# rlorenzo/facet

Hardware: AMD Instinct MI355X
Metric: images/sec whole-node (TOPIQ+SAMP+CLIP+InsightFace ensemble), 1024² batch (higher is better)
Workload: dtype f32

## Files before the change

### facet_amd/_lib.py

```python
import ctypes as C
import importlib.util
import os
import sys
import threading

import numpy as np

_HERE = os.path.dirname(os.path.abspath(__file__))
LIB_PATH = os.environ.get("FACET_AMD_LIB") or os.path.join(_HERE, "libfacet_engine.so")

FE_MODEL_TOPIQ, FE_MODEL_CLIP, FE_MODEL_SAMP, FE_MODEL_U2NETP, FE_MODEL_AESTHETIC, FE_MODEL_VLM = range(6)
FE_MODEL_SCRFD, FE_MODEL_ARCFACE = 5, 6
FE_RECORD_FLOATS = 789
FE_GRAPH_FACE_DET, FE_GRAPH_FACE_LMK, FE_GRAPH_FACE_REC = 0, 1, 2
FE_FACE_FLOATS = 739
FE_STATS_DOUBLES = 264
FILTERS = {"lanczos": 1, "bilinear": 2, "bicubic": 3}
FE_PRECISION_RES32 = 16
FE_PRECISION_SPLIT3 = 32
PRECISION = {"f32": 0, "fp32": 0, "float32": 0, "bf16": 1, "bfloat16": 1, "f16": 2, "fp16": 2, "float16": 2, "half": 2,
             "bf16+r32": 1 | FE_PRECISION_RES32, "f16+r32": 2 | FE_PRECISION_RES32, "f16x3": 2 | FE_PRECISION_RES32 | FE_PRECISION_SPLIT3}
PRECISION_NAME = {0: "f32", 1: "bf16", 2: "f16", 1 | FE_PRECISION_RES32: "bf16+r32", 2 | FE_PRECISION_RES32: "f16+r32",
                  2 | FE_PRECISION_RES32 | FE_PRECISION_SPLIT3: "f16x3"}
ACT = {"none": 0, None: 0, "relu": 1, "gelu": 2, "sigmoid": 3, "softplus": 5}


class EngineError(RuntimeError):
    pass


class EngineCapacityError(EngineError):
    """The batch did not fit (device memory, arena, KV cache): FE_ERR_CAPACITY, raised by the padded-batch image path only
    (vlm_preprocess_rgb, vlm_encode_preprocessed, vlm_prefill with pad). Fewer images at a time may fit. jpeg_encode / face_thumbnails raise it when the
    caller's `cap` is too small for an image."""


FE_ERR_CAPACITY = -4


_lib = None
_lib_lock = threading.Lock()

_f32p = C.POINTER(C.c_float)
_u8p = C.POINTER(C.c_uint8)
_i64p = C.POINTER(C.c_int64)

SIGNATURES = {
    "fe_create": (C.c_int, [C.c_int, C.c_size_t, C.POINTER(C.c_void_p)]),
    "fe_destroy": (None, [C.c_void_p]),
    "fe_last_error": (C.c_char_p, [C.c_void_p]),
    "fe_version": (C.c_char_p, []),
    "fe_sync": (C.c_int, [C.c_void_p]),
    "fe_set_microbatch": (C.c_int, [C.c_void_p, C.c_int]),
    "fe_set_precision": (C.c_int, [C.c_void_p, C.c_int]),
    "fe_model_precision": (C.c_int, [C.c_void_p, C.c_int]),
    "fe_dev_alloc": (C.c_int, [C.c_void_p, C.c_size_t, C.POINTER(C.c_void_p)]),
    "fe_dev_free": (C.c_int, [C.c_void_p, C.c_void_p]),
    "fe_memcpy_h2d": (C.c_int, [C.c_void_p, C.c_void_p, C.c_void_p, C.c_size_t]),
    "fe_memcpy_d2h": (C.c_int, [C.c_void_p, C.c_void_p, C.c_void_p, C.c_size_t]),
    "fe_timer_start": (C.c_int, [C.c_void_p]),
    "fe_timer_stop": (C.c_int, [C.c_void_p, _f32p]),
    "fe_profile_enable": (C.c_int, [C.c_void_p, C.c_int]),
    "fe_profile_count": (C.c_int, [C.c_void_p]),
    "fe_profile_get": (C.c_int, [C.c_void_p, C.c_int, C.c_char_p, C.c_int, C.POINTER(C.c_double),
                                 C.POINTER(C.c_double), _f32p]),
    "fe_flops_reset": (C.c_int, [C.c_void_p]),
    "fe_flops_get": (C.c_int, [C.c_void_p, C.POINTER(C.c_double)]),
    "fe_flops_get_executed": (C.c_int, [C.c_void_p, C.POINTER(C.c_double)]),
    "fe_flops_get_half": (C.c_int, [C.c_void_p, C.POINTER(C.c_double)]),
    "fe_weights_begin": (C.c_int, [C.c_void_p, C.c_int]),
    "fe_weights_set": (C.c_int, [C.c_void_p, C.c_int, C.c_char_p, _f32p, _i64p, C.c_int]),
    "fe_weights_commit": (C.c_int, [C.c_void_p, C.c_int]),
    "fe_model_unload": (C.c_int, [C.c_void_p, C.c_int]),
    "fe_model_loaded": (C.c_int, [C.c_void_p, C.c_int]),
    "fe_op_conv2d": (C.c_int, [C.c_void_p, _f32p, C.c_int, C.c_int, C.c_int, C.c_int, _f32p, C.c_int, C.c_int,
                               C.c_int, _f32p, _f32p, _f32p, C.c_int, C.c_int, C.c_int, C.c_int, C.c_int, _f32p]),
    "fe_op_topiq_gate64": (C.c_int, [C.c_void_p, _f32p, C.c_int, C.c_int, C.c_int, _f32p, _f32p, _f32p, _f32p, _f32p, C.c_float,
                                     _f32p, _f32p, C.c_int, C.c_int, _f32p]),
    "fe_op_conv3x3_c64": (C.c_int, [C.c_void_p, _f32p, C.c_int, C.c_int, C.c_int, _f32p, _f32p, _f32p, C.c_int, _f32p, _f32p, _f32p,
                                    _f32p, _f32p]),
    "fe_op_maxpool2d": (C.c_int, [C.c_void_p, _f32p, C.c_int, C.c_int, C.c_int, C.c_int, C.c_int, C.c_int,
                                  C.c_int, C.c_int, _f32p]),
    "fe_op_bilinear": (C.c_int, [C.c_void_p, _f32p, C.c_int, C.c_int, C.c_int, C.c_int, C.c_int, C.c_int, _f32p]),
    "fe_op_adaptive_avgpool": (C.c_int, [C.c_void_p, _f32p, C.c_int, C.c_int, C.c_int, C.c_int, C.c_int, C.c_int,
                                         _f32p]),
    "fe_op_layernorm": (C.c_int, [C.c_void_p, _f32p, C.c_int, C.c_int, _f32p, _f32p, C.c_float, _f32p]),
    "fe_op_vlm_select": (C.c_int, [C.c_void_p, _f32p, C.c_int, C.c_int, C.POINTER(C.c_int32), _f32p]),
    "fe_set_conv_variant": (C.c_int, [C.c_void_p, C.c_int]),
    "fe_bench_conv": (C.c_int, [C.c_void_p] + [C.c_int] * 12 + [_f32p]),
    "fe_topiq_configure": (C.c_int, [C.c_void_p, C.c_int, C.c_int]),
    "fe_topiq_f32_below": (C.c_int, [C.c_void_p, C.c_longlong]),
    "fe_topiq_feature_shape": (C.c_int, [C.c_int, C.c_int, C.c_int, C.POINTER(C.c_int)]),
    "fe_ensemble_select": (C.c_int, [C.c_void_p, C.c_int]),
    "fe_ensemble_score_dev": (C.c_int, [C.c_void_p, C.c_void_p, C.c_int, C.c_int, C.c_int, C.c_int, C.c_void_p, C.c_int,
                                        C.POINTER(C.c_int)]),
    "fe_topiq_features": (C.c_int, [C.c_void_p, C.c_void_p, C.c_int, C.c_int, C.c_int, C.c_int, C.c_int, _f32p]),
    "fe_topiq_score": (C.c_int, [C.c_void_p, C.c_void_p, C.c_int, C.c_int, C.c_int, C.c_int, _f32p]),
    "fe_clip_encode_image": (C.c_int, [C.c_void_p, C.c_void_p, C.c_int, C.c_int, _f32p, _f32p, _f32p]),
    "fe_resize_u8": (C.c_int, [C.c_void_p, C.c_void_p, C.c_int, C.c_int, C.c_int, C.c_int, C.c_int, C.c_int, C.c_int,
                               C.c_void_p]),
    "fe_clip_encode_images": (C.c_int, [C.c_void_p, C.c_void_p, C.c_int, C.c_int, C.c_int, C.c_int, _f32p, _f32p, _f32p]),
    "fe_samp_score_images": (C.c_int, [C.c_void_p, C.c_void_p, C.c_int, C.c_int, C.c_int, C.c_int, C.c_int, _f32p,
                                       _f32p, _f32p]),
    "fe_clip_encode_text": (C.c_int, [C.c_void_p, C.POINTER(C.c_int32), C.c_int, C.c_int, _f32p]),
    "fe_tag_similarities": (C.c_int, [C.c_void_p, _f32p, C.c_int, _f32p, C.c_int, C.c_int, _f32p]),
    "fe_vlm_configure": (C.c_int, [C.c_void_p, C.c_int, C.c_int, C.c_int, C.c_float, C.c_float, C.POINTER(C.c_int)]),
    "fe_vlm_dims": (C.c_int, [C.c_void_p, C.POINTER(C.c_int)]),
    "fe_vlm_prefill": (C.c_int, [C.c_void_p, C.POINTER(C.c_int32), C.POINTER(C.c_int32), C.c_int, C.c_int, C.c_int, C.POINTER(C.c_int32), _f32p]),
    "fe_vlm_decode_step": (C.c_int, [C.c_void_p, C.POINTER(C.c_int32), C.POINTER(C.c_int32), C.c_int, C.POINTER(C.c_int32), _f32p]),
    "fe_vlm_vision_configure": (C.c_int, [C.c_void_p, C.c_int, C.POINTER(C.c_int), C.c_int]),
    "fe_vlm_encode_images": (C.c_int, [C.c_void_p, _f32p, C.c_int, C.POINTER(C.c_int32), C.POINTER(C.c_int32), C.POINTER(C.c_int32), C.c_int,
                                       C.POINTER(C.c_int32), C.c_int, _f32p]),
    "fe_vlm_prefill_images": (C.c_int, [C.c_void_p, C.POINTER(C.c_int32), C.POINTER(C.c_int32), C.c_int, C.c_int, C.c_int, C.POINTER(C.c_int32), C.c_int,
                                        C.POINTER(C.c_int32), _f32p]),
    "fe_vlm_generate": (C.c_int, [C.c_void_p, C.POINTER(C.c_int32), C.POINTER(C.c_int32), C.c_int, C.c_int, C.POINTER(C.c_int32)]),
    "fe_vlm_generate_scored": (C.c_int, [C.c_void_p, C.POINTER(C.c_int32), C.POINTER(C.c_int32), C.c_int, C.c_int, C.POINTER(C.c_int32), _f32p]),
    "fe_vlm_last_logprobs": (C.c_int, [C.c_void_p, _f32p]),
    "fe_vlm_preprocess_rgb": (C.c_int, [C.c_void_p, C.c_void_p, C.c_int, C.POINTER(C.c_int32), _f32p, _f32p, _f32p]),
    "fe_vlm_encode_preprocessed": (C.c_int, [C.c_void_p, C.POINTER(C.c_int32), C.POINTER(C.c_int32), C.POINTER(C.c_int32), C.c_int,
                                             C.POINTER(C.c_int32), C.c_int, _f32p]),
    "fe_vlm_vision_dims": (C.c_int, [C.c_void_p, C.POINTER(C.c_int)]),
    "fe_vlm3_configure": (C.c_int, [C.c_void_p, C.c_int, C.c_int, C.c_int, C.c_float, C.c_float, C.POINTER(C.c_int), C.c_int, C.POINTER(C.c_int), C.c_int]),
    "fe_vlm3_encode_images": (C.c_int, [C.c_void_p, _f32p, C.c_int, C.POINTER(C.c_int32), C.POINTER(C.c_int32), _f32p, C.POINTER(C.c_int32), C.c_int, _f32p, _f32p]),
    "fe_vlm2_configure": (C.c_int, [C.c_void_p, C.c_int, C.c_int, C.c_int, C.c_float, C.c_float, C.POINTER(C.c_int), C.c_int]),
    "fe_vlm2_encode_images": (C.c_int, [C.c_void_p, _f32p, C.c_int, C.POINTER(C.c_int32), C.POINTER(C.c_int32), C.c_int, _f32p]),
    "fe_vlm_generate_until": (C.c_int, [C.c_void_p, C.POINTER(C.c_int32), C.POINTER(C.c_int32), C.c_int, C.c_int, C.POINTER(C.c_int32), C.c_int, C.c_int,
                                        C.POINTER(C.c_int32), _f32p, C.POINTER(C.c_int)]),
    "fe_vlm_prefill_images_padded": (C.c_int, [C.c_void_p, C.POINTER(C.c_int32), C.POINTER(C.c_int32), C.c_int, C.c_int, C.c_int, C.POINTER(C.c_int32),
                                               C.POINTER(C.c_int32), C.c_int, C.POINTER(C.c_int32), _f32p]),
    "fe_ensemble_score": (C.c_int, [C.c_void_p, C.c_void_p, C.c_int, C.c_int, C.c_int, C.c_int, _f32p,
                                    C.POINTER(C.c_int)]),
    "fe_u2netp_saliency": (C.c_int, [C.c_void_p, _f32p, C.c_int, C.c_int, C.c_int, _f32p]),
    "fe_samp_forward": (C.c_int, [C.c_void_p, _f32p, C.c_int, _f32p, _f32p, _f32p, _f32p]),
    "fe_onnx_probe": (C.c_int, [C.c_void_p, C.c_size_t, C.POINTER(C.c_int), C.POINTER(C.c_int), C.POINTER(C.c_int), _i64p,
                                C.c_char_p, C.c_int]),
    "fe_graph_load": (C.c_int, [C.c_void_p, C.c_int, C.c_void_p, C.c_size_t]),
    "fe_graph_unload": (C.c_int, [C.c_void_p, C.c_int]),
    "fe_graph_loaded": (C.c_int, [C.c_void_p, C.c_int]),
    "fe_graph_info": (C.c_int, [C.c_void_p, C.c_int, C.POINTER(C.c_int), C.POINTER(C.c_int), _i64p, C.POINTER(C.c_int)]),
    "fe_graph_run": (C.c_int, [C.c_void_p, C.c_int, C.c_void_p, C.c_int, C.c_int, C.c_int, C.c_int, C.c_int]),
    "fe_graph_output_info": (C.c_int, [C.c_void_p, C.c_int, C.c_int, C.c_char_p, C.c_int, _i64p, C.POINTER(C.c_int)]),
    "fe_graph_output_copy": (C.c_int, [C.c_void_p, C.c_int, C.c_int, _f32p, C.c_size_t]),
    "fe_face_detect": (C.c_int, [C.c_void_p, C.c_void_p, C.c_int, C.c_int, C.c_int, C.c_int, C.c_int, C.c_int, C.c_float, C.c_int,
                                 _f32p, C.POINTER(C.c_int), _f32p]),
    "fe_face_crops_run": (C.c_int, [C.c_void_p, C.c_int, C.c_void_p, C.c_int, C.c_int, C.c_int, C.c_int, C.c_int, C.POINTER(C.c_int),
                                    C.POINTER(C.c_double), C.c_int, C.c_float, C.c_float, C.c_int, _f32p, C.c_int, C.c_void_p]),
    "fe_face_analyze": (C.c_int, [C.c_void_p, C.c_void_p, C.c_int, C.c_int, C.c_int, C.c_int, C.c_int, C.c_int, C.c_float, C.c_float,
                                  C.c_int, _f32p, C.POINTER(C.c_int), C.POINTER(C.c_int)]),
    "fe_image_stats": (C.c_int, [C.c_void_p, C.c_void_p, C.c_int, C.c_int, C.c_int, C.c_int, C.POINTER(C.c_double), C.c_void_p, C.c_void_p]),
    "fe_roi_laplacian": (C.c_int, [C.c_void_p, C.c_void_p, C.c_int, C.c_int, C.c_int, C.c_int, C.c_int, C.POINTER(C.c_int), C.POINTER(C.c_int),
                                   C.POINTER(C.c_double)]),
    "fe_cv_resize_linear_u8": (C.c_int, [C.c_void_p, C.c_void_p, C.c_int, C.c_int, C.c_int, C.c_int, C.c_int, C.c_void_p]),
    "fe_aesthetic_score": (C.c_int, [C.c_void_p, C.POINTER(C.c_float), C.c_int, C.POINTER(C.c_float)]),
    "fe_swap_rb_u8": (C.c_int, [C.c_void_p, C.c_void_p, C.c_int, C.c_size_t, C.c_void_p]),
    "fe_leading_lines": (C.c_int, [C.c_void_p, C.c_void_p, C.c_int, C.c_int, C.c_int, C.c_int, C.c_int, C.c_int, C.c_int, C.c_int, C.c_int, C.c_int,
                                   C.c_void_p, C.c_void_p, C.c_void_p]),
    "fe_external_contours": (C.c_int, [C.c_void_p, C.c_void_p, C.c_int, C.c_int, C.c_int, C.c_int, C.c_longlong, C.c_int, C.c_void_p, C.c_void_p]),
    "fe_subject_region": (C.c_int, [C.c_void_p, C.c_void_p, C.c_int, C.c_int, C.c_int, C.c_int, C.c_int, C.c_void_p, C.c_void_p, C.c_void_p,
                                    C.c_void_p]),
    "fe_phash": (C.c_int, [C.c_void_p, C.c_void_p, C.c_int, C.c_int, C.c_int, C.c_int, C.c_int, C.c_void_p, C.c_void_p, C.c_void_p]),
    "fe_resize_u8_box": (C.c_int, [C.c_void_p, C.c_void_p, C.c_int, C.c_int, C.c_int, C.c_int, C.c_int, C.c_int, C.c_void_p, C.c_int, C.c_void_p]),
# ... 213 lines not shown
    def timer_stop(self):
        ms = C.c_float()
        self._ck(self.lib.fe_timer_stop(self.h, C.byref(ms)))
        return ms.value

    def profile_enable(self, on=True):
        self._ck(self.lib.fe_profile_enable(self.h, 1 if on else 0))

    def profile_records(self):
        out = []
        n = self.lib.fe_profile_count(self.h)
        buf = C.create_string_buffer(160)
        for i in range(n):
            fl, by, ms = C.c_double(), C.c_double(), C.c_float()
            self._ck(self.lib.fe_profile_get(self.h, i, buf, 160, C.byref(fl), C.byref(by), C.byref(ms)))
            out.append({"name": buf.value.decode(), "flops": fl.value, "bytes": by.value, "ms": ms.value})
        return out

    def flops_executed(self):
        f = C.c_double()
        self._ck(self.lib.fe_flops_get_executed(self.h, C.byref(f)))
        return f.value

    def flops_half(self):
        f = C.c_double()
        self._ck(self.lib.fe_flops_get_half(self.h, C.byref(f)))
        return f.value

    def flops_reset(self):
        self._ck(self.lib.fe_flops_reset(self.h))

    def flops(self):
        v = C.c_double()
        self._ck(self.lib.fe_flops_get(self.h, C.byref(v)))
        return v.value

    def load_weights(self, model, state_dict):
        self._ck(self.lib.fe_weights_begin(self.h, model))
        for name, t in state_dict.items():
            a = t.detach().cpu().numpy() if hasattr(t, "detach") else np.asarray(t)
            if a.dtype.kind not in "fiu" or a.ndim > 6:
                continue
            a, ap = _f32(a)
            shape = (C.c_int64 * max(a.ndim, 1))(*a.shape)
            self._ck(self.lib.fe_weights_set(self.h, model, name.encode(), ap, shape, a.ndim))
        self._ck(self.lib.fe_weights_commit(self.h, model))

    def unload(self, model):
        self._ck(self.lib.fe_model_unload(self.h, model))

    def loaded(self, model):
        return bool(self.lib.fe_model_loaded(self.h, model))

    def conv2d(self, x, w, scale=None, shift=None, res=None, res_after_act=False, stride=1, pad=0, dil=1, act=None):
        x, xp = _f32(x)
        w, wp = _f32(w)
        n, c, h, ww = x.shape
        cout, cin, kh, kw = w.shape
        assert cin == c
        ho = (h + 2 * pad - dil * (kh - 1) - 1) // stride + 1
        wo = (ww + 2 * pad - dil * (kw - 1) - 1) // stride + 1
        y = np.empty((n, cout, ho, wo), np.float32)
        sp = hp = rp = None
        if scale is not None:
            scale, sp = _f32(scale)
        if shift is not None:
            shift, hp = _f32(shift)
        if res is not None:
            res, rp = _f32(res)
        self._ck(self.lib.fe_op_conv2d(self.h, xp, n, c, h, ww, wp, cout, kh, kw, sp, hp, rp, int(res_after_act),
                                       stride, pad, dil, ACT[act], y.ctypes.data_as(_f32p)))
        return y

    def topiq_gate64(self, x, w0, b0, w2, b2, w4, b4, wx, bx, wblk_act="gelu", gate_act="gelu"):
        x, xp = _f32(x)
        n, c, h, w = x.shape
        assert c == 64
        arrs = [_f32(a) for a in (w0, b0, w2, b2, w4, wx, bx)]
        y = np.empty((n, 64, h // 16, w // 16), np.float32)
        self._ck(self.lib.fe_op_topiq_gate64(self.h, xp, n, h, w, arrs[0][1], arrs[1][1], arrs[2][1], arrs[3][1], arrs[4][1], C.c_float(float(b4)),
                                             arrs[5][1], arrs[6][1], ACT[wblk_act], ACT[gate_act], y.ctypes.data_as(_f32p)))
        return y

    def conv3x3_c64(self, x, w2, scale2=None, shift2=None, act2="relu", w3=None, scale3=None, shift3=None, res=None):
        x, xp = _f32(x)
        n, c, h, w = x.shape
        assert c == 64
        keep = [_f32(a) if a is not None else (None, None) for a in (w2, scale2, shift2, w3, scale3, shift3, res)]
        y = np.empty((n, 256 if w3 is not None else 64, h, w), np.float32)
        self._ck(self.lib.fe_op_conv3x3_c64(self.h, xp, n, h, w, keep[0][1], keep[1][1], keep[2][1], ACT[act2], keep[3][1], keep[4][1], keep[5][1],
                                            keep[6][1], y.ctypes.data_as(_f32p)))
        return y

    def maxpool2d(self, x, k, stride, pad=0, ceil_mode=False):
        x, xp = _f32(x)
        n, c, h, w = x.shape

        def od(i):
            if ceil_mode:
                o = -(-(i + 2 * pad - k) // stride) + 1
                if (o - 1) * stride >= i + pad:
                    o -= 1
                return o
            return (i + 2 * pad - k) // stride + 1
        y = np.empty((n, c, od(h), od(w)), np.float32)
        self._ck(self.lib.fe_op_maxpool2d(self.h, xp, n, c, h, w, k, stride, pad, int(ceil_mode),
                                          y.ctypes.data_as(_f32p)))
        return y

    def bilinear(self, x, ho, wo):
        x, xp = _f32(x)
        n, c, h, w = x.shape
        y = np.empty((n, c, ho, wo), np.float32)
        self._ck(self.lib.fe_op_bilinear(self.h, xp, n, c, h, w, ho, wo, y.ctypes.data_as(_f32p)))
        return y

    def adaptive_avgpool(self, x, ho, wo):
        x, xp = _f32(x)
        n, c, h, w = x.shape
        y = np.empty((n, c, ho, wo), np.float32)
        self._ck(self.lib.fe_op_adaptive_avgpool(self.h, xp, n, c, h, w, ho, wo, y.ctypes.data_as(_f32p)))
        return y

    def layernorm(self, x, g, b, eps=1e-5):
        x, xp = _f32(x)
        g, gp = _f32(g)
        b, bp = _f32(b)
        rows, d = x.shape
        y = np.empty_like(x)
        self._ck(self.lib.fe_op_layernorm(self.h, xp, rows, d, gp, bp, eps, y.ctypes.data_as(_f32p)))
        return y

    def set_conv_variant(self, v):
        self._ck(self.lib.fe_set_conv_variant(self.h, int(v)))

    def bench_conv(self, n, h, w, cin, cout, k, stride=1, pad=0, res=False, act="relu", variant=0, iters=10):
        ms = C.c_float()
        self._ck(self.lib.fe_bench_conv(self.h, n, h, w, cin, cout, k, stride, pad, int(res), ACT[act], variant, iters,
                                        C.byref(ms)))
        return ms.value

    @staticmethod
    def _img_ptr(images):
        if isinstance(images, tuple):
            p, n, h, w = images
            return p, n, h, w, 1, None
        a = np.ascontiguousarray(images, dtype=np.uint8)
        assert a.ndim == 4 and a.shape[3] == 3
        return a.ctypes.data_as(C.c_void_p), a.shape[0], a.shape[1], a.shape[2], 0, a

    def topiq_configure(self, gate_act="gelu", weight_blk_act="gelu"):
        self._ck(self.lib.fe_topiq_configure(self.h, ACT[gate_act], ACT[weight_blk_act]))

    def topiq_f32_below(self, pixels):
        self._ck(self.lib.fe_topiq_f32_below(self.h, int(pixels)))

    def topiq_feature_shape(self, h, w, level):
        dims = (C.c_int * 3)()
        if self.lib.fe_topiq_feature_shape(int(h), int(w), int(level), dims) != 0:
            raise EngineError(f"topiq_feature_shape: bad arguments h={h} w={w} level={level}")
        return tuple(dims)

    def topiq_features(self, images, level):
        p, n, h, w, dev, keep = self._img_ptr(images)
        y = np.empty((n,) + self.topiq_feature_shape(h, w, level), np.float32)
        self._ck(self.lib.fe_topiq_features(self.h, p, n, h, w, dev, level, y.ctypes.data_as(_f32p)))
# ... 803 lines not shown
```

### facet_amd/csrc/capi.hip

```cpp
#include "../../include/facet_engine.h"
#include <thread>

#include "engine.h"
#include <type_traits>
#include "lines_host.h"
#include "onnx_graph.h"
#include <algorithm>
#include <cmath>
#include <tuple>
#include <cstring>
#include <stdexcept>

using namespace fe;

struct fe_ctx {
  Ctx c;
  hipEvent_t t0 = nullptr, t1 = nullptr;
  int microbatch = 8;
  hipStream_t copy_stream = nullptr;
  uint8_t* stage_buf[2] = {nullptr, nullptr};
  size_t stage_cap[2] = {0, 0};
  hipEvent_t ev_copied[2] = {nullptr, nullptr}, ev_consumed[2] = {nullptr, nullptr};
  short* warp_wtab = nullptr;
  int* hsv_sdiv = nullptr; int* hsv_hdiv = nullptr;
// ... 502 lines not shown
}

int fe_op_conv2d(fe_ctx* ctx, const float* x, int n, int c, int h, int w, const float* weight, int cout, int kh, int kw,
                 const float* scale, const float* shift, const float* res, int res_after_act, int stride, int pad,
                 int dil, int act, float* y) {
  FE_API_BEGIN(ctx)
  Ctx& C = ctx->c;
  FE_CHECK(x && weight && y && n > 0 && c > 0 && h > 0 && w > 0 && cout > 0 && kh > 0 && kw > 0 && stride > 0 && dil > 0,
           "bad conv arguments");
  C.arena.reset();
  DeviceWeights dw;
  dw.prec = C.precision;
  WeightStore ws;
  const int64_t wshape[4] = {cout, c, kh, kw};
  ws.set("w.weight", weight, wshape, 4);
  ConvW cw = build_conv(dw, ws, "w", "", false);
  std::vector<float> v;
  if (scale) { v.assign(scale, scale + cout); cw.scale = dw.upload(v); }
  if (shift) { v.assign(shift, shift + cout); cw.shift = dw.upload(v); }
  const int ho = conv_out_dim(h, kh, stride, pad, dil), wo = conv_out_dim(w, kw, stride, pad, dil);
  FE_CHECK(ho > 0 && wo > 0, "conv output is empty");
  auto half_op = [&](auto* tag) {
    typedef std::remove_pointer_t<decltype(tag)> E;
    FE_CHECK(cw.wh, "fe_op_conv2d(2-byte): Cin must be a multiple of 8 (16 for spatial kernels)");
    TensorT<E> xt = upload_nchw<E>(C, x, n, c, h, w, cw.CinPadH);
    ConvOptsT<E> o;
    o.sh = o.sw = stride; o.ph = o.pw = pad; o.dh = o.dw = dil; o.act = act; o.res_after_act = res_after_act;
    TensorT<E> rt;
    if (C.res32) {
      Tensor r32, y32 = C.arena.tensor(n, ho, wo, cout);
      if (res) { r32 = upload_nchw(C, res, n, cout, ho, wo, cout); o.res32 = &r32; }
      o.y32 = &y32;
      TensorT<E> yt = C.arena.tensor_t<E>(n, ho, wo, cout);
      conv_forward(C, cw, xt, yt, o);
      download_nchw(C, y32, cout, y);
      std::vector<float> y16((size_t)n * cout * ho * wo);
      download_nchw(C, yt, cout, y16.data());
      for (size_t i = 0; i < y16.size(); ++i) {
        const float a = std::fmin(std::fmax(y[i], -65504.f), 65504.f);
        FE_CHECK(std::fabs(y16[i] - a) <= std::fabs(a) * (PrecOf<E>::value == PREC_F16 ? 4.9e-4f : 3.95e-3f) + 6.2e-5f,
                 "fe_op_conv2d(res32): 2-byte output %g is not the rounding of the fp32 output %g at %zu", y16[i], y[i], i);
      }
      return;
    }
    if (res) { rt = upload_nchw<E>(C, res, n, cout, ho, wo, cout); o.res = &rt; }
    TensorT<E> yt = conv_new(C, cw, xt, o);
    download_nchw(C, yt, cout, y);
  };
  if (C.precision == PREC_BF16) {
    half_op((bf16*)nullptr);
  } else if (C.precision == PREC_F16) {
    half_op((f16*)nullptr);
  } else {
    Tensor xt = upload_nchw(C, x, n, c, h, w, cw.CinPad);
    ConvOpts o;
    o.sh = o.sw = stride; o.ph = o.pw = pad; o.dh = o.dw = dil; o.act = act; o.res_after_act = res_after_act;
    Tensor rt;
    if (res) { rt = upload_nchw(C, res, n, cout, ho, wo, cout); o.res = &rt; }
    Tensor yt = conv_new(C, cw, xt, o);
    download_nchw(C, yt, cout, y);
  }
  FE_API_END(ctx)
}

int fe_op_topiq_gate64(fe_ctx* ctx, const float* x, int n, int h, int w, const float* w0, const float* b0, const float* w2, const float* b2,
                       const float* w4, float b4, const float* wx, const float* bx, int wblk_act, int gate_act, float* y) {
  FE_API_BEGIN(ctx)
  Ctx& C = ctx->c;
  FE_CHECK(x && w0 && b0 && w2 && b2 && w4 && wx && bx && y && n > 0 && h > 0 && w > 0 && h % 16 == 0 && w % 16 == 0, "bad gate64 arguments");
  FE_CHECK(C.precision == PREC_BF16 || C.precision == PREC_F16, "fe_op_topiq_gate64: the fused gate exists for the 2-byte element types only");
  C.arena.reset();
  DeviceWeights dw;
  dw.prec = C.precision;
  GatedConvW g;
  build_gate64_fragments(dw, g, w0, b0, w2, b2, w4, b4, wx, bx);
  auto run = [&](auto* tag) {
    typedef std::remove_pointer_t<decltype(tag)> E;
    TensorT<E> xt = upload_nchw<E>(C, x, n, 64, h, w, 64);
    TensorT<E> yt = C.arena.tensor_t<E>(n, h / 16, w / 16, 64);
    launch_topiq_gate64(xt, yt, g.fused, g.fused_bias, wblk_act, gate_act, C.stream);
    download_nchw(C, yt, 64, y);
  };
  if (C.precision == PREC_BF16) run((bf16*)nullptr); else run((f16*)nullptr);
  FE_API_END(ctx)
}

int fe_op_conv3x3_c64(fe_ctx* ctx, const float* x, int n, int h, int w, const float* w2, const float* scale2, const float* shift2, int act2,
                      const float* w3, const float* scale3, const float* shift3, const float* res, float* y) {
  FE_API_BEGIN(ctx)
  Ctx& C = ctx->c;
  FE_CHECK(x && w2 && y && n > 0 && h > 0 && w > 0 && (!w3 || res), "bad conv3x3_c64 arguments");
  FE_CHECK(C.precision == PREC_BF16 || C.precision == PREC_F16, "fe_op_conv3x3_c64: the halo-tiled kernel exists for the 2-byte element types only");
  C.arena.reset();
  DeviceWeights dw;
  dw.prec = C.precision;
  void *f2 = nullptr, *f3 = nullptr;
  build_c64_fragments(dw, w2, w3, &f2, &f3);
  std::vector<float> v;
  auto up = [&](const float* a, int cnt) -> float* { if (!a) return nullptr; v.assign(a, a + cnt); return dw.upload(v); };
  float *s2 = up(scale2, 64), *h2 = up(shift2, 64), *s3 = up(scale3, 256), *h3 = up(shift3, 256);
  const int cout = w3 ? 256 : 64;
  auto run = [&](auto* tag) {
    typedef std::remove_pointer_t<decltype(tag)> E;
    TensorT<E> xt = upload_nchw<E>(C, x, n, 64, h, w, 64);
    TensorT<E> yt = C.arena.tensor_t<E>(n, h, w, cout);
    TensorT<E> rt;
    if (w3) rt = upload_nchw<E>(C, res, n, 256, h, w, 256);
    launch_conv3x3_c64(xt, yt, w3 ? &rt : nullptr, f2, f3, s2, h2, s3, h3, act2, C.stream);
    download_nchw(C, yt, cout, y);
  };
  if (C.precision == PREC_BF16) run((bf16*)nullptr); else run((f16*)nullptr);
  FE_API_END(ctx)
}

int fe_op_maxpool2d(fe_ctx* ctx, const float* x, int n, int c, int h, int w, int k, int stride, int pad, int ceil_mode,
                    float* y) {
  FE_API_BEGIN(ctx)
  Ctx& C = ctx->c;
  C.arena.reset();
  Tensor xt = upload_nchw(C, x, n, c, h, w, c);
  auto od = [&](int in) {
    int o = ceil_mode ? (in + 2 * pad - k + stride - 1) / stride + 1 : (in + 2 * pad - k) / stride + 1;
    if (ceil_mode && (o - 1) * stride >= in + pad) --o;
    return o;
  };
  Tensor yt = C.arena.tensor(n, od(h), od(w), c);
  launch_maxpool(xt, yt, k, stride, pad, C.stream);
  download_nchw(C, yt, c, y);
  FE_API_END(ctx)
}

int fe_op_bilinear(fe_ctx* ctx, const float* x, int n, int c, int h, int w, int ho, int wo, float* y) {
  FE_API_BEGIN(ctx)
  Ctx& C = ctx->c;
  C.arena.reset();
  Tensor xt = upload_nchw(C, x, n, c, h, w, c);
  Tensor yt = C.arena.tensor(n, ho, wo, c);
  launch_bilinear(xt, yt, C.stream);
  download_nchw(C, yt, c, y);
  FE_API_END(ctx)
}

int fe_op_adaptive_avgpool(fe_ctx* ctx, const float* x, int n, int c, int h, int w, int ho, int wo, float* y) {
  FE_API_BEGIN(ctx)
  Ctx& C = ctx->c;
  C.arena.reset();
  Tensor xt = upload_nchw(C, x, n, c, h, w, c);
  Tensor yt = C.arena.tensor(n, ho, wo, c);
  launch_adaptive_avgpool(xt, yt, C.stream);
  download_nchw(C, yt, c, y);
  FE_API_END(ctx)
}

int fe_op_layernorm(fe_ctx* ctx, const float* x, int rows, int d, const float* g, const float* b, float eps, float* y) {
  FE_API_BEGIN(ctx)
  Ctx& C = ctx->c;
  C.arena.reset();
  const size_t bytes = (size_t)rows * d * sizeof(float);
  float* dx = (float*)C.arena.alloc(bytes);
  float* dy = (float*)C.arena.alloc(bytes);
  float* dg = (float*)C.arena.alloc(d * sizeof(float));
  float* db = (float*)C.arena.alloc(d * sizeof(float));
  FE_HIP(hipMemcpyAsync(dx, x, bytes, hipMemcpyHostToDevice, C.stream));
  FE_HIP(hipMemcpyAsync(dg, g, d * sizeof(float), hipMemcpyHostToDevice, C.stream));
  FE_HIP(hipMemcpyAsync(db, b, d * sizeof(float), hipMemcpyHostToDevice, C.stream));
  launch_layernorm(dx, d, dy, d, dg, db, rows, d, eps, C.stream);
// ... 2168 lines not shown
```

### facet_amd/csrc/engine.h

```cpp
#pragma once
#include "fe_common.h"
#include "../../include/facet_engine.h"
#include <memory>
#include <tuple>

namespace fe {

struct HostTensor {
  std::vector<float> data;
  std::vector<int64_t> shape;
  size_t numel() const { size_t n = 1; for (auto d : shape) n *= (size_t)d; return n; }
};

class WeightStore {
 public:
  void clear() { t_.clear(); }
  void set(const std::string& name, const float* data, const int64_t* shape, int ndim);
  bool has(const std::string& name) const { return t_.count(name) != 0; }
  const HostTensor& get(const std::string& name) const;
  size_t size() const { return t_.size(); }
 private:
  std::map<std::string, HostTensor> t_;
};

// ... 17 lines not shown
  ConvW w;
};

struct LayerNormW {
  float* g = nullptr; float* b = nullptr; int d = 0; float eps = 1e-5f;
};

enum Precision : int { PREC_F32 = 0, PREC_BF16 = 1, PREC_F16 = 2 };
constexpr int PREC_RES32_FLAG = 16;
constexpr int PREC_SPLIT3_FLAG = 32;
template <class T> struct PrecOf { static constexpr int value = PREC_F32; };
template <> struct PrecOf<bf16> { static constexpr int value = PREC_BF16; };
template <> struct PrecOf<f16> { static constexpr int value = PREC_F16; };
inline uint16_t f32_to_bf16_bits(float f) {
  uint32_t u; memcpy(&u, &f, 4);
  if ((u & 0x7FFFFFFFu) > 0x7F800000u) return (uint16_t)((u >> 16) | 0x40);
  return (uint16_t)((u + 0x7FFFu + ((u >> 16) & 1u)) >> 16);
}
inline uint16_t f32_to_f16_bits(float f) {
  uint32_t u; memcpy(&u, &f, 4);
  const uint32_t sign = (u >> 16) & 0x8000u;
  u &= 0x7FFFFFFFu;
  if (u > 0x7F800000u) return (uint16_t)(sign | 0x7E00u);
  if (u >= 0x477FF000u) return (uint16_t)(sign | 0x7BFFu);
  if (u < 0x38800000u) {
    if (u < 0x33000000u) return (uint16_t)sign;
    const int shift = 126 - (int)(u >> 23);
    const uint32_t m = (u & 0x7FFFFFu) | 0x800000u;
    const uint32_t h = m >> shift, rem = m & ((1u << shift) - 1), half = 1u << (shift - 1);
    return (uint16_t)(sign | (h + ((rem > half || (rem == half && (h & 1))) ? 1 : 0)));
  }
  const uint32_t h = ((u - 0x38000000u) >> 13), rem = u & 0x1FFFu;
  return (uint16_t)(sign | (h + ((rem > 0x1000u || (rem == 0x1000u && (h & 1))) ? 1 : 0)));
}
inline uint16_t f32_to_half_bits(float f, int prec) { return prec == PREC_F16 ? f32_to_f16_bits(f) : f32_to_bf16_bits(f); }
void pack_conv_bf16(DeviceWeights& dw, const HostTensor& w, ConvW& c);

ConvW pack_conv(DeviceWeights& dw, const HostTensor& w, const std::vector<float>* scale, const std::vector<float>* shift);
ConvW build_conv(DeviceWeights& dw, const WeightStore& ws, const std::string& conv_prefix,
                 const std::string& bn_prefix, bool conv_bias, float bn_eps = 1e-5f);
ConvW build_linear(DeviceWeights& dw, const WeightStore& ws, const std::string& prefix, bool bias);
ConvW build_linear_rows(DeviceWeights& dw, const HostTensor& w, const HostTensor* b, int row0, int rows);
LayerNormW build_ln(DeviceWeights& dw, const WeightStore& ws, const std::string& prefix, float eps = 1e-5f);

struct Ctx;

struct MHAW {
  ConvW q, k;
  float* wv = nullptr;
  void* wv_h = nullptr;
  float* bv = nullptr;
  ConvW out;
  int d = 0, heads = 0;
};
MHAW build_mha(DeviceWeights& dw, const WeightStore& ws, const std::string& prefix, int heads);
template <class T, class RT>
void mha_forward(Ctx& c, const MHAW& m, const T* q_in, int ldq, const T* kv_in, int ldkv, int B, int Lq,
                 int Lk, const RT* res, int ldr, RT* y, int ldy, bool causal = false);
void linear_forward(Ctx& c, const ConvW& w, const float* x, int ldx, int M, float* y, int ldy, int act,
                    const float* res = nullptr, int ldr = 0);
void linear_forward(Ctx& c, const ConvW& w, const bf16* x, int ldx, int M, bf16* y, int ldy, int act,
                    const bf16* res = nullptr, int ldr = 0);
void linear_forward(Ctx& c, const ConvW& w, const f16* x, int ldx, int M, f16* y, int ldy, int act,
                    const f16* res = nullptr, int ldr = 0);
void linear_forward_s32(Ctx& c, const ConvW& w, const bf16* x, int ldx, int M, float* y, int ldy, int act, const float* res = nullptr, int ldr = 0);
void linear_forward_s32(Ctx& c, const ConvW& w, const f16* x, int ldx, int M, float* y, int ldy, int act, const float* res = nullptr, int ldr = 0);
void linear_forward_res(Ctx& c, const ConvW& w, const float* x, int ldx, int M, float* y, int ldy, int act, const float* res, int ldr);
void linear_forward_res(Ctx& c, const ConvW& w, const bf16* x, int ldx, int M, bf16* y, int ldy, int act, const bf16* res, int ldr);
void linear_forward_res(Ctx& c, const ConvW& w, const f16* x, int ldx, int M, f16* y, int ldy, int act, const f16* res, int ldr);
void linear_forward_res(Ctx& c, const ConvW& w, const bf16* x, int ldx, int M, float* y, int ldy, int act, const float* res, int ldr);
void linear_forward_res(Ctx& c, const ConvW& w, const f16* x, int ldx, int M, float* y, int ldy, int act, const float* res, int ldr);
void linear_forward_f32(Ctx& c, const ConvW& w, const float* x, int ldx, int M, float* y, int ldy, int act);
void linear_forward_f32(Ctx& c, const ConvW& w, const bf16* x, int ldx, int M, float* y, int ldy, int act);
void linear_forward_f32(Ctx& c, const ConvW& w, const f16* x, int ldx, int M, float* y, int ldy, int act);
void linear_forward_xf32(Ctx& c, const ConvW& w, int prec, const float* x, int ldx, int M, float* y, int ldy, int act);
template <class T>
inline TensorT<T> mat_view(const T* p, int rows, int cols, int ld) {
  TensorT<T> t; t.p = const_cast<T*>(p); t.n = 1; t.h = 1; t.w = rows; t.c = cols; t.ld = ld; return t;
}

void conv_forward(Ctx& c, const ConvW& w, const Tensor& x, const Tensor& y, const ConvOpts& o);
void conv_forward(Ctx& c, const ConvW& w, const TensorH& x, const TensorH& y, const ConvOptsT<bf16>& o);
void conv_forward(Ctx& c, const ConvW& w, const TensorF16& x, const TensorF16& y, const ConvOptsT<f16>& o);
template <class T>
TensorT<T> conv_new(Ctx& c, const ConvW& w, const TensorT<T>& x, const ConvOptsT<T>& o);
template <class T>
TensorT<T> first_conv(Ctx& c, const ConvW& w, const Tensor& x, const ConvOpts& o);
inline int conv_out_dim(int in, int k, int s, int p, int d) { return (in + 2 * p - d * (k - 1) - 1) / s + 1; }

struct ResBlock {
  ConvW c1, c2, c3, down;
  bool has_down = false, bottleneck = true;
  int stride = 1;
  void* frag2 = nullptr;
  void* frag3 = nullptr;
};
float* build_n16_weights(DeviceWeights& dw, const float* W, int cin);
void launch_conv3x3_n16_f32(const Tensor& x, const Tensor& y, const float* wt, const float* scale, const float* shift, int act, hipStream_t s);
void build_c64_fragments(DeviceWeights& dw, const float* W2, const float* W3, void** frag2, void** frag3);
template <class E>
void launch_conv3x3_c64(const TensorT<E>& x, const TensorT<E>& y, const TensorT<E>* res, const void* frag2, const void* frag3, const float* scale2, const float* shift2,
                        const float* scale3, const float* shift3, int act2, hipStream_t s);
struct ResNet {
  ConvW stem;
  std::vector<std::vector<ResBlock>> layers;
  bool bottleneck = true;
};
void build_resnet(ResNet& r, DeviceWeights& dw, const WeightStore& ws, const std::string& prefix,
                  bool bottleneck, const int blocks[4], bool seq_names);
template <class T>
TensorT<T> resnet_forward(Ctx& c, const ResNet& r, const Tensor& x_nhwc4, std::vector<TensorT<T>>* feats, bool res32 = false, Tensor* last32 = nullptr);

enum ResizeFilter : int { FE_FILTER_LANCZOS = 1, FE_FILTER_BILINEAR = 2, FE_FILTER_BICUBIC = 3 };
struct ResizeCoeffs { std::vector<int> kk, bounds; int ksize = 0, out = 0; };
struct ResizeCoeffsDev { int* kk = nullptr; int* bounds = nullptr; int ksize = 0; };
void build_resize_coeffs(int in_size, int out_size, int filter, ResizeCoeffs& rc);
void build_resize_coeffs(int in_size, float in0, float in1, int out_size, int filter, ResizeCoeffs& rc);
constexpr int FE_FILTER_KEY_PHASH = -1;
struct Ctx;
const ResizeCoeffsDev& upload_resize_coeffs(Ctx& c, const std::tuple<int, int, int>& key, const ResizeCoeffs& rc);
void resize_u8(Ctx& c, const uint8_t* d_src, int n, int h, int w, int oh, int ow, int filter, int y0, int ch, int x0,
               int cw, uint8_t* d_dst);
void resize_u8_box(Ctx& c, const uint8_t* d_src, int n, int h, int w, int oh, int ow, int filter, const float box[4], uint8_t* d_dst);

void reduce_u8(Ctx& c, const uint8_t* d_src, int n, int h, int w, int fx, int fy, const int box[4], uint8_t* d_dst);
size_t jpeg_bound(int h, int w);
size_t jpeg_scratch_bytes(int h, int w);
void launch_jpeg_encode(Ctx& c, const uint8_t* d_img, int n, int h, int w, int bgr, int quality, uint8_t* d_out, size_t cap, int32_t* d_lengths);
bool face_thumbnails(Ctx& c, const uint8_t* d_bgr, int n, int h, int w, int m, const int32_t* img_index, const int32_t* crops, const int32_t* out_sizes,
                     int quality, uint8_t* out, size_t cap, int32_t* lengths);

void jpeg_probe(const uint8_t* data, size_t len, int flags, int32_t out[10]);
void jpeg_scaled_size(int h, int w, int scale, int* sh, int* sw);
void jpeg_decode_batch(Ctx& c, const uint8_t* const* data, const size_t* len, int n, int h, int w, int scale, int bgr, int apply_orientation, int dst_on_device, int flags,
                       uint8_t* dst, int32_t* status);

void phash_cos_table(double* out);
size_t phash_tmp_bytes(int n, int h);
void launch_phash(Ctx& c, const uint8_t* d_img, int n, int h, int w, int bgr, uint8_t* d_tmp, const double* d_cos, uint64_t* d_hashes,
                  uint8_t* d_small, double* d_dct);
void launch_hamming_pairs(const uint64_t* d_hashes, int n, int maxd, int64_t cap, int* d_pairs, unsigned long long* d_count, hipStream_t s);

int cluster_max_rounds(int n);
void cluster_core_distances(Ctx& c, const float* x, int n, int d, int on_device, int normalise, int k, double* core, int32_t* core_idx);
void cluster_mreach_mst(Ctx& c, const float* x, int n, int d, int on_device, int normalise, int k, int32_t* edge_u, int32_t* edge_v,
                        double* edge_w, double* core, int32_t* rounds_out);
void cluster_best_match(Ctx& c, const float* q, int nq, const float* cc, int nc, int d, float* best_sim, int32_t* best_idx);
void similar_topk(Ctx& c, const fe_sim_rows& q, const fe_sim_rows& cand, int d, int cosine, const float* w, const int32_t* q_self, const uint8_t* visible,
                  int k, int32_t* idx, float* score);
void similar_pairs(Ctx& c, const fe_sim_rows& q, const fe_sim_rows& cand, int d, int cosine, const float* w, const int32_t* q_self, const uint8_t* visible,
                   const float* thr, int n_thr, int upper, int64_t max_pairs, int32_t* pairs, float* scores, int64_t* count);

class Graph;
struct GraphSlot;

struct VlmConfig {
  int n_heads = 28, n_kv_heads = 4, head_dim = 128; float rope_theta = 1e6f, rms_eps = 1e-6f; int mrope[3] = {16, 24, 24};
  int vis_heads = 16, fullatt[8] = {7, 15, 23, 31, 0, 0, 0, 0}, n_fullatt = 4;
  bool qwen3 = false; int deepstack[8] = {0, 0, 0, 0, 0, 0, 0, 0}, n_deepstack = 0;
  bool qwen2 = false;
};

struct OpTiming { std::string name; double flops; double bytes; float ms; };

struct Ctx {
  int device = 0;
  hipStream_t stream = nullptr;
  Arena arena;
  std::string err;
  std::mutex mu;
  bool profile = false;
  std::vector<OpTiming> timings;
  double flops_accum = 0.0;
  double flops_saved = 0.0;
  double flops_half = 0.0;
  int force_variant = 0;
  int precision = PREC_F32;
  bool res32 = false;
  bool split3 = false;
  int topiq_gate_act = ACT_GELU, topiq_wblk_act = ACT_GELU;
  size_t topiq_f32_below = 0;

  std::map<std::tuple<int, int, int>, ResizeCoeffsDev> resize_cache;
  std::map<std::tuple<int, int, int, uint32_t, uint32_t>, ResizeCoeffsDev> resize_box_cache;
  std::map<std::tuple<int, int, int>, void*> jpeg_cache;
  void* jpegdec_stage = nullptr;
  size_t jpegdec_stage_cap = 0;
  WeightStore staging[8];
  std::unique_ptr<struct TopiqModel> topiq;
  std::unique_ptr<struct U2NetPModel> u2netp;
  std::unique_ptr<struct SampModel> samp;
  std::unique_ptr<struct ClipModel> clip;
  std::unique_ptr<struct AestheticModel> aesthetic;
  std::unique_ptr<struct ClipTextModel> clip_text;
  std::unique_ptr<struct VlmModel> vlm;
  VlmConfig vlm_cfg;
  std::unique_ptr<GraphSlot> graphs[8];
  ~Ctx();
};

struct EncLayerW { MHAW attn; ConvW lin1, lin2; LayerNormW n1, n2; };
struct DecLayerW { MHAW cross; ConvW lin1, lin2; LayerNormW n1, n2, n3; };
struct GatedConvW {
  ConvW split_x1, w0, w2, w4;
  void* fused = nullptr;
  float* fused_bias = nullptr;
  void* w2_frag = nullptr;
};
void build_gate64_fragments(DeviceWeights& dw, GatedConvW& g, const float* W0, const float* B0, const float* W2, const float* B2, const float* W4, float b4,
                            const float* Wx, const float* Bx);
template <class E>
void launch_topiq_gate64(const TensorT<E>& x, const TensorT<E>& out, const void* frag, const float* bias, int wblk_act, int gate_act, hipStream_t s);

struct TopiqModel {
  DeviceWeights dw;
  ResNet backbone;
  bool has_head = false;
  int gate_act = ACT_GELU;
  int wblk_act = ACT_GELU;
  GatedConvW gate[5];
  ConvW dim_reduce[5];
  EncLayerW sa[5];
  DecLayerW cross[4];
  EncLayerW pool;
  LayerNormW s_ln0, s_ln3;
  ConvW s_l1, s_l4, s_l6;
  std::vector<float> h_emb, w_emb;
  std::map<std::pair<int, int>, float*> pos;
};
struct RSUW {
  ConvW in;
  std::vector<ConvW> enc;
  std::vector<ConvW> dec;
  int depth = 0;
  bool dilated = false;
};
struct U2NetPModel {
  DeviceWeights dw;
  RSUW stage[11];
  ConvW side[6], outconv;
};
struct SampModel {
  DeviceWeights dw;
  ResNet backbone;
  ConvW pattern_weight, pattern[8], att_feat, att_pred, com0, com3, com5;
};
void build_u2netp(U2NetPModel& m, const WeightStore& ws);
void build_sampnet(SampModel& m, const WeightStore& ws);
template <class T>
void u2netp_forward(Ctx& c, const U2NetPModel& m, const Tensor& x_nhwc4, const TensorT<T>& sal);
template <class T, class TS>
void sampnet_forward(Ctx& c, const SampModel& m, const Tensor& x_nhwc4, const TensorT<TS>& sal, float* pw, float* attrs,
                     float* dist);

struct ClipBlockW {
  LayerNormW ln1, ln2; MHAW attn; ConvW fc, proj;
  ConvW qkv3, out2, fc3, proj3;
};
struct ClipModel {
  DeviceWeights dw;
  ConvW patch, proj;
  float* pos = nullptr; float* cls = nullptr;
  LayerNormW ln_pre, ln_post;
  std::vector<ClipBlockW> blocks;
  int width = 0, heads = 0, tokens = 0, patch_size = 0, out_dim = 0;
  bool split3 = false;
  float* zero_bias = nullptr;
};
struct AestheticModel { DeviceWeights dw; ConvW l0, l2; };
struct ClipTextModel {
  DeviceWeights dw;
  float* tok_emb = nullptr;
  float* pos = nullptr;
  std::vector<ClipBlockW> blocks;
  LayerNormW ln_final;
  ConvW proj;
  int vocab = 0, width = 0, ctx = 0, heads = 0, out_dim = 0;
};
void build_clip_text(ClipTextModel& m, const WeightStore& ws);
void clip_text_forward(Ctx& c, const ClipTextModel& m, const int* tokens, const int* eot, int B, float* feat);
void build_clip(ClipModel& m, const WeightStore& ws);
void build_aesthetic(AestheticModel& m, const WeightStore& ws);
template <class T, class RT = T>
void clip_forward(Ctx& c, const ClipModel& m, const Tensor& x_nhwc4, float* feat);
void clip_forward_split3(Ctx& c, const ClipModel& m, const Tensor& x_nhwc4, float* feat);
void aesthetic_forward(Ctx& c, const AestheticModel& m, const float* feat, int B, float* raw);
void l2_normalize(Ctx& c, const float* x, float* y, int rows, int d);

struct VlmLayerW { ConvW qkv, o, gate, up, down; bf16* ln1 = nullptr; bf16* ln2 = nullptr; bf16* qn = nullptr; bf16* kn = nullptr; };
struct VlmVisionBlockW { ConvW qkv, proj, gate, up, down; bf16* n1 = nullptr; bf16* n2 = nullptr; };
struct VlmVisionW {
  bool present = false;
  ConvW patch, m0, m2;
  std::vector<VlmVisionBlockW> blocks;
  bf16* ln_q = nullptr; float* inv_freq = nullptr;
// ... 73 lines not shown
```

### facet_amd/csrc/engine.hip

```cpp
#include "engine.h"
#include "onnx_graph.h"
#include <algorithm>
#include <cmath>
#include <cstdlib>

namespace fe {

void WeightStore::set(const std::string& name, const float* data, const int64_t* shape, int ndim) {
  HostTensor h;
  h.shape.assign(shape, shape + ndim);
  h.data.assign(data, data + h.numel());
  t_[name] = std::move(h);
}
const HostTensor& WeightStore::get(const std::string& name) const {
  auto it = t_.find(name);
  if (it == t_.end()) throw Error("missing weight tensor '" + name + "'");
  return it->second;
}

float* DeviceWeights::upload(const std::vector<float>& v) {
  void* p = nullptr;
  const size_t b = v.size() * sizeof(float);
  FE_HIP(hipMalloc(&p, b ? b : 16));
  if (b) FE_HIP(hipMemcpy(p, v.data(), b, hipMemcpyHostToDevice));
// ... 125 lines not shown
  const int K = ntaps * c.CinPadH;
  c.KpH = (K + CONV_KALIGN_H - 1) / CONV_KALIGN_H * CONV_KALIGN_H;
  std::vector<uint16_t> packed((size_t)c.Cout * c.KpH, 0);
  for (int co = 0; co < c.Cout; ++co)
    for (int ci = 0; ci < c.Cin; ++ci)
      for (int t = 0; t < ntaps; ++t) {
        const size_t k = ntaps > 1 ? ((size_t)(ci / c.cb) * ntaps + t) * c.cb + (ci % c.cb) : (size_t)ci;
        packed[(size_t)co * c.KpH + k] = f32_to_half_bits(w.data[((size_t)co * c.Cin + ci) * ntaps + t], dw.prec);
      }
  c.wh = dw.upload_raw(packed.data(), packed.size() * sizeof(uint16_t));
  c.hprec = dw.prec;
  if (c.Cout <= 2 && ntaps > 1) {
    const int T = ntaps * c.Cout, T8 = (T + 7) & ~7;
    c.KpTH = (c.CinPadH + CONV_KALIGN_H - 1) / CONV_KALIGN_H * CONV_KALIGN_H;
    std::vector<uint16_t> tp((size_t)T8 * c.KpTH, 0);
    for (int t = 0; t < ntaps; ++t)
      for (int co = 0; co < c.Cout; ++co)
        for (int ci = 0; ci < c.Cin; ++ci)
          tp[(size_t)(t * c.Cout + co) * c.KpTH + ci] = f32_to_half_bits(w.data[((size_t)co * c.Cin + ci) * ntaps + t], dw.prec);
    c.wtap_h = dw.upload_raw(tp.data(), tp.size() * sizeof(uint16_t));
  }
}

ConvW build_conv(DeviceWeights& dw, const WeightStore& ws, const std::string& conv_prefix,
                 const std::string& bn_prefix, bool conv_bias, float bn_eps) {
  const HostTensor& w = ws.get(conv_prefix + ".weight");
  const int cout = (int)w.shape[0];
  std::vector<float> scale, shift;
  const bool bn = !bn_prefix.empty();
  if (bn) {
    const auto& g = ws.get(bn_prefix + ".weight").data;
    const auto& b = ws.get(bn_prefix + ".bias").data;
    const auto& mu = ws.get(bn_prefix + ".running_mean").data;
    const auto& var = ws.get(bn_prefix + ".running_var").data;
    FE_CHECK((int)g.size() == cout && (int)var.size() == cout, "bn %s size mismatch", bn_prefix.c_str());
    scale.resize(cout); shift.resize(cout);
    for (int i = 0; i < cout; ++i) {
      const float inv = 1.0f / std::sqrt(var[i] + bn_eps);
      scale[i] = g[i] * inv;
      float sh = b[i] - mu[i] * scale[i];
      if (conv_bias) sh += ws.get(conv_prefix + ".bias").data[i] * scale[i];
      shift[i] = sh;
    }
  } else if (conv_bias) {
    shift = ws.get(conv_prefix + ".bias").data;
    FE_CHECK((int)shift.size() == cout, "bias %s size mismatch", conv_prefix.c_str());
  }
  return pack_conv(dw, w, scale.empty() ? nullptr : &scale, shift.empty() ? nullptr : &shift);
}

ConvW build_linear(DeviceWeights& dw, const WeightStore& ws, const std::string& prefix, bool bias) {
  const HostTensor& w = ws.get(prefix + ".weight");
  FE_CHECK(w.shape.size() == 2, "linear %s weight rank", prefix.c_str());
  if (bias) {
    const auto& b = ws.get(prefix + ".bias").data;
    return pack_conv(dw, w, nullptr, &b);
  }
  return pack_conv(dw, w, nullptr, nullptr);
}

ConvW build_linear_rows(DeviceWeights& dw, const HostTensor& w, const HostTensor* b, int row0, int rows) {
  FE_CHECK(w.shape.size() == 2 && row0 + rows <= w.shape[0], "linear_rows: bad range");
  HostTensor sub;
  const int in = (int)w.shape[1];
  sub.shape = {rows, in};
  sub.data.assign(w.data.begin() + (size_t)row0 * in, w.data.begin() + (size_t)(row0 + rows) * in);
  if (b) {
    std::vector<float> bb(b->data.begin() + row0, b->data.begin() + row0 + rows);
    return pack_conv(dw, sub, nullptr, &bb);
  }
  return pack_conv(dw, sub, nullptr, nullptr);
}

LayerNormW build_ln(DeviceWeights& dw, const WeightStore& ws, const std::string& prefix, float eps) {
  LayerNormW l;
  const auto& g = ws.get(prefix + ".weight").data;
  l.d = (int)g.size();
  l.g = dw.upload(g);
  l.b = dw.upload(ws.get(prefix + ".bias").data);
  l.eps = eps;
  return l;
}

void conv_forward(Ctx& c, const ConvW& w, const Tensor& x, const Tensor& y, const ConvOpts& o) {
  FE_CHECK(x.c == w.CinPad, "conv: input channels %d != packed Cin %d", x.c, w.CinPad);
  FE_CHECK(y.c == w.Cout && y.n == x.n, "conv: output view mismatch (c=%d Cout=%d)", y.c, w.Cout);
  ConvParams p{};
  p.x = x.p; p.ldx = x.ld;
  p.w = w.w; p.scale = w.scale; p.shift = w.shift; p.slope = w.slope;
  FE_CHECK(o.act != ACT_PRELU || w.slope, "conv: PReLU without slopes");
  if (o.res) {
    FE_CHECK(o.res->c == y.c && o.res->pixels() == y.pixels(), "conv: residual shape mismatch");
    p.res = o.res->p; p.ldr = o.res->ld;
  }
  if (o.gate) {
    FE_CHECK(o.gate->pixels() == y.pixels() && (o.gate->c == 1 || o.gate->c == y.c), "conv: gate shape mismatch");
    p.gate = o.gate->p; p.ldg = o.gate->ld; p.gate_c1 = o.gate->c == 1;
  }
  p.y = y.p; p.ldy = y.ld;
  p.N = x.n; p.H = x.h; p.W = x.w; p.Cin = w.CinPad;
  p.Ho = y.h; p.Wo = y.w; p.Cout = w.Cout;
  p.KH = w.KH; p.KW = w.KW; p.sh = o.sh; p.sw = o.sw; p.ph = o.ph; p.pw = o.pw; p.dh = o.dh; p.dw = o.dw;
  FE_CHECK(y.h == conv_out_dim(x.h, w.KH, o.sh, o.ph, o.dh) && y.w == conv_out_dim(x.w, w.KW, o.sw, o.pw, o.dw),
           "conv: output dims %dx%d inconsistent with input %dx%d", y.h, y.w, x.h, x.w);
  p.K = w.K; p.Kp = w.Kp;
  p.M = (int)y.pixels();
  FE_CHECK(y.pixels() < (1ull << 31), "conv: M too large");
  p.act = o.act; p.res_after_act = o.res_after_act;
  p.variant = c.force_variant;
  if (w.wtap && o.act != ACT_PRELU && o.sh == 1 && o.sw == 1 && !o.res && !o.gate && p.variant == 0 && y.h == x.h && y.w == x.w) {
    const int T = w.KH * w.KW * w.Cout, Tp = (T + 3) & ~3;
    const size_t mark = c.arena.mark();
    Tensor z = c.arena.tensor(x.n, x.h, x.w, Tp);
    ConvParams q{};
    q.x = x.p; q.ldx = x.ld; q.w = w.wtap; q.y = z.p; q.ldy = Tp;
    q.N = x.n; q.H = x.h; q.W = x.w; q.Cin = w.CinPad; q.Ho = x.h; q.Wo = x.w; q.Cout = T;
    q.KH = q.KW = 1; q.sh = q.sw = q.dh = q.dw = 1;
    q.K = w.CinPad; q.Kp = w.KpT; q.M = (int)x.pixels();
    launch_conv(q, c.stream);
    launch_tap_gather(z.p, Tp, x.n, x.h, x.w, w.KH, w.KW, o.ph, o.pw, o.dh, o.dw, w.Cout, w.scale, w.shift, o.act, y.p,
                      y.ld, y.h, y.w, c.stream);
    c.arena.rewind(mark);
    c.flops_accum += 2.0 * p.M * (double)(w.KH * w.KW * w.Cin) * (w.CoutAlg ? w.CoutAlg : p.Cout);
    return;
  }
  static const bool no_wino = getenv("FE_NO_WINO") != nullptr;
  const bool wino_plain = !o.res && (o.act == ACT_NONE || o.act == ACT_RELU);
  if (w.wino && !no_wino && p.variant == 0 && o.sh == 1 && o.sw == 1 && o.ph == 1 && o.pw == 1 && o.dh == 1 && o.dw == 1 &&
      !o.gate && (wino_plain || (w.wino_m == 4 && (o.act == ACT_NONE || o.act == ACT_RELU || o.act == ACT_PRELU))) && y.h == x.h && y.w == x.w && (((uintptr_t)x.p | (uintptr_t)y.p) & 15) == 0 &&
      x.ld % 4 == 0 && y.ld % 4 == 0) {
    const int ts = w.wino_m, planes = (ts + 2) * (ts + 2);
    const int th = (x.h + ts - 1) / ts, tw = (x.w + ts - 1) / ts;
    const size_t tiles = (size_t)x.n * th * tw;
    const size_t wino_bytes = (size_t)planes * tiles * ((size_t)w.CinPad + w.Cout) * sizeof(float) + 1024;
    if (tiles < (1u << 30) / 36 && c.arena.mark() + wino_bytes <= c.arena.capacity()) {
      const size_t mark = c.arena.mark();
      float* V = (float*)c.arena.alloc((size_t)planes * tiles * w.CinPad * sizeof(float));
      float* Mb = (float*)c.arena.alloc((size_t)planes * tiles * w.Cout * sizeof(float));
      hipEvent_t e0 = nullptr, e1 = nullptr;
      if (c.profile) {
        FE_HIP(hipEventCreate(&e0)); FE_HIP(hipEventCreate(&e1));
        FE_HIP(hipEventRecord(e0, c.stream));
      }
      if (ts == 2) launch_wino_input(x, th, tw, V, c.stream);
      else launch_wino4_input(x, th, tw, V, c.stream);
      ConvParams g{};
      g.x = V; g.ldx = w.CinPad; g.w = w.wino; g.ldw = w.CinPad; g.y = Mb; g.ldy = w.Cout;
      g.M = (int)tiles; g.K = w.CinPad; g.Cout = w.Cout;
      g.N = 1; g.H = 1; g.W = g.M; g.Ho = 1; g.Wo = g.M; g.KH = g.KW = 1; g.sh = g.sw = g.dh = g.dw = 1;
      g.Kp = w.CinPad; g.Cin = w.CinPad;
      g.batch = planes; g.nb1 = 1; g.xs2 = (long long)tiles * w.CinPad; g.ws2 = (long long)w.Cout * w.CinPad; g.ys2 = (long long)tiles * w.Cout;
      launch_conv(g, c.stream);
      if (ts == 2) launch_wino_output(Mb, y, th, tw, w.scale, w.shift, o.act == ACT_RELU, c.stream);
      else launch_wino4_output(Mb, y, th, tw, w.scale, w.shift, o.act, w.slope, o.res, o.res_after_act, c.stream);
      if (c.profile) {
        FE_HIP(hipEventRecord(e1, c.stream));
        FE_HIP(hipEventSynchronize(e1));
        float ms = 0.f;
        FE_HIP(hipEventElapsedTime(&ms, e0, e1));
        (void)hipEventDestroy(e0); (void)hipEventDestroy(e1);
        char nm[128];
        snprintf(nm, sizeof nm, "wino3x3 M=%d K=%d N=%d", p.M, p.K, p.Cout);
        c.timings.push_back({nm, 2.0 * p.M * (double)(9 * w.Cin) * p.Cout, 0.0, ms});
      }
      c.arena.rewind(mark);
      c.flops_accum += 2.0 * p.M * (double)(w.KH * w.KW * w.Cin) * (w.CoutAlg ? w.CoutAlg : p.Cout);
      c.flops_saved += 2.0 * p.M * (double)(9 * w.Cin) * (w.CoutAlg ? w.CoutAlg : p.Cout) - 2.0 * (double)planes * (double)tiles * w.CinPad * w.Cout;
      return;
    }
  }
  static const bool no_splitk = getenv("FE_NO_SPLITK") != nullptr;
  if (!no_splitk && w.KH == 1 && w.KW == 1 && o.sh == 1 && o.sw == 1 && o.ph == 0 && o.pw == 0 && !o.gate && p.variant == 0 && p.M <= 256 &&
      w.CinPad >= (getenv("FE_SPLITK_MIN") ? atoi(getenv("FE_SPLITK_MIN")) : 2048) && w.K == w.CinPad &&
      (o.act == ACT_NONE || o.act == ACT_RELU || o.act == ACT_PRELU)) {
    int splits = 0;
    for (int s = 64; s >= 2; --s)
      if (w.CinPad % s == 0 && (w.CinPad / s) % 32 == 0 && w.CinPad / s >= 256) { splits = s; break; }
    const size_t part_bytes = (size_t)splits * p.M * w.Cout * sizeof(float);
    if (splits && c.arena.mark() + part_bytes + 1024 <= c.arena.capacity()) {
      const size_t mark = c.arena.mark();
      float* part = (float*)c.arena.alloc(part_bytes);
      const int Ks = w.CinPad / splits;
      hipEvent_t e0 = nullptr, e1 = nullptr;
      if (c.profile) {
        FE_HIP(hipEventCreate(&e0)); FE_HIP(hipEventCreate(&e1));
        FE_HIP(hipEventRecord(e0, c.stream));
      }
      ConvParams g{};
      g.x = x.p; g.ldx = x.ld; g.w = w.w; g.ldw = w.Kp; g.y = part; g.ldy = w.Cout;
      g.M = p.M; g.K = Ks; g.Kp = Ks; g.Cin = Ks; g.Cout = w.Cout;
      g.N = 1; g.H = 1; g.W = g.M; g.Ho = 1; g.Wo = g.M; g.KH = g.KW = 1; g.sh = g.sw = g.dh = g.dw = 1;
      g.batch = splits; g.nb1 = 1; g.xs2 = Ks; g.ws2 = Ks; g.ys2 = (long long)p.M * w.Cout;
      launch_conv(g, c.stream);
      launch_splitk_reduce(part, splits, p.M, w.Cout, w.scale, w.shift, w.slope, o.act, o.res ? o.res->p : nullptr, o.res ? o.res->ld : 0,
                           o.res_after_act, y.p, y.ld, c.stream);
      if (c.profile) {
        FE_HIP(hipEventRecord(e1, c.stream));
        FE_HIP(hipEventSynchronize(e1));
        float ms = 0.f;
        FE_HIP(hipEventElapsedTime(&ms, e0, e1));
        (void)hipEventDestroy(e0); (void)hipEventDestroy(e1);
        char nm[128];
        snprintf(nm, sizeof nm, "splitk%d 1x1 M=%d K=%d N=%d", splits, p.M, p.K, p.Cout);
        c.timings.push_back({nm, 2.0 * p.M * (double)w.Cin * (w.CoutAlg ? w.CoutAlg : p.Cout), 0.0, ms});
      }
      c.arena.rewind(mark);
      c.flops_accum += 2.0 * p.M * (double)w.Cin * (w.CoutAlg ? w.CoutAlg : p.Cout);
      return;
    }
  }
  static const bool no_stem = getenv("FE_NO_STEM") != nullptr;
  const bool stem = w.wstem && !no_stem && p.variant == 0 && o.sh == o.sw && o.ph == w.KH / 2 && o.pw == w.KW / 2 && o.dh == 1 && o.dw == 1 && !o.res &&
                    !o.gate && (o.act == ACT_NONE || o.act == ACT_RELU || o.act == ACT_PRELU);
  auto launch = [&]() {
    if (stem && launch_stem(x.p, x.ld, x.n, x.h, x.w, w.wstem, w.scale, w.shift, w.slope, w.Cout, w.KH, o.sh,
                            o.act == ACT_RELU ? 1 : (o.act == ACT_PRELU ? 2 : 0), y.p, y.ld, y.h, y.w, c.stream))
      return;
    launch_conv(p, c.stream);
  };
  if (c.profile) {
    hipEvent_t e0, e1;
    FE_HIP(hipEventCreate(&e0)); FE_HIP(hipEventCreate(&e1));
    FE_HIP(hipEventRecord(e0, c.stream));
    launch();
    FE_HIP(hipEventRecord(e1, c.stream));
    FE_HIP(hipEventSynchronize(e1));
    float ms = 0.f;
    FE_HIP(hipEventElapsedTime(&ms, e0, e1));
    (void)hipEventDestroy(e0); (void)hipEventDestroy(e1);
    char nm[128];
    snprintf(nm, sizeof nm, "conv%dx%d s%d d%d M=%d K=%d N=%d", w.KH, w.KW, o.sh, o.dh, p.M, p.K, p.Cout);
    double bytes = 4.0 * ((double)x.pixels() * x.c + (double)y.pixels() * y.c * (o.res ? 2 : 1) + (double)w.Cout * w.K);
    c.timings.push_back({nm, 2.0 * p.M * (double)(w.KH * w.KW * w.Cin) * (w.CoutAlg ? w.CoutAlg : p.Cout), bytes, ms});
  } else {
    launch();
  }
  c.flops_accum += 2.0 * p.M * (double)(w.KH * w.KW * w.Cin) * (w.CoutAlg ? w.CoutAlg : p.Cout);
}

template <class E>
static void conv_forward_half(Ctx& c, const ConvW& w, const TensorT<E>& x, const TensorT<E>& y, const ConvOptsT<E>& o) {
  if (!w.wh && w.w && PrecOf<E>::value != PREC_F32 && !o.res && !o.gate && x.ld == x.c && y.ld == y.c && x.c >= w.CinPad) {
    const size_t mark = c.arena.mark();
    Tensor xf = c.arena.tensor(x.n, x.h, x.w, x.c), yf = c.arena.tensor(y.n, y.h, y.w, y.c);
    launch_convert(x.p, xf.p, x.numel(), c.stream);
    ConvOpts of; of.sh = o.sh; of.sw = o.sw; of.ph = o.ph; of.pw = o.pw; of.dh = o.dh; of.dw = o.dw; of.act = o.act;
    conv_forward(c, w, xf.slice(0, w.CinPad), yf, of);
    launch_convert(yf.p, y.p, y.numel(), c.stream);
    c.arena.rewind(mark);
    return;
  }
  FE_CHECK(w.wh && w.hprec == PrecOf<E>::value, "conv(2-byte): this layer has no weights of the activations' type (model committed under another "
           "precision, or a 3-channel first layer)");
  FE_CHECK(x.c == w.CinPadH, "conv(bf16): input channels %d != packed Cin %d", x.c, w.CinPadH);
  FE_CHECK(y.c == w.Cout && y.n == x.n, "conv(bf16): output view mismatch (c=%d Cout=%d)", y.c, w.Cout);
  FE_CHECK(y.p || o.y32, "conv(2-byte): no output tensor");
  FE_CHECK(y.h == conv_out_dim(x.h, w.KH, o.sh, o.ph, o.dh) && y.w == conv_out_dim(x.w, w.KW, o.sw, o.pw, o.dw),
           "conv(bf16): output dims %dx%d inconsistent with input %dx%d", y.h, y.w, x.h, x.w);
  FE_CHECK(y.pixels() < (1ull << 31), "conv: M too large");
  const double flops = 2.0 * (double)y.pixels() * (double)(w.KH * w.KW * w.Cin) * (w.CoutAlg ? w.CoutAlg : w.Cout);
  hipEvent_t e0 = nullptr, e1 = nullptr;
  if (c.profile) {
    FE_HIP(hipEventCreate(&e0)); FE_HIP(hipEventCreate(&e1));
    FE_HIP(hipEventRecord(e0, c.stream));
  }
  ConvParamsT<E> p{};
  p.scale = w.scale; p.shift = w.shift; p.slope = w.slope;
  p.N = x.n; p.H = x.h; p.W = x.w; p.Cin = w.CinPadH; p.x = x.p; p.ldx = x.ld;
  if (w.wtap_h && o.act != ACT_PRELU && o.sh == 1 && o.sw == 1 && !o.res && !o.gate && !o.res32 && !o.y32 && y.h == x.h && y.w == x.w) {
    const int T = w.KH * w.KW * w.Cout, T8 = (T + 7) & ~7;
    const size_t mark = c.arena.mark();
    TensorT<E> z = c.arena.tensor_t<E>(x.n, x.h, x.w, T8);
    p.w = (const E*)w.wtap_h; p.y = z.p; p.ldy = T8; p.scale = p.shift = p.slope = nullptr;
    p.Ho = x.h; p.Wo = x.w; p.Cout = T8; p.KH = p.KW = 1; p.sh = p.sw = p.dh = p.dw = 1;
    p.K = w.CinPadH; p.Kp = w.KpTH; p.M = (int)x.pixels(); p.cb = 32;
    launch_conv_bf16(p, c.stream);
    launch_tap_gather(z.p, T8, x.n, x.h, x.w, w.KH, w.KW, o.ph, o.pw, o.dh, o.dw, w.Cout, w.scale, w.shift, o.act, y.p, y.ld, y.h, y.w, c.stream);
    c.arena.rewind(mark);
  } else {
    FE_CHECK(o.act != ACT_PRELU || w.slope, "conv: PReLU without slopes");
    if (o.res) {
      FE_CHECK(o.res->c == y.c && o.res->pixels() == y.pixels(), "conv: residual shape mismatch");
      p.res = o.res->p; p.ldr = o.res->ld;
    }
    if (o.gate) {
      FE_CHECK(o.gate->pixels() == y.pixels() && (o.gate->c == 1 || o.gate->c == y.c), "conv: gate shape mismatch");
      p.gate = o.gate->p; p.ldg = o.gate->ld; p.gate_c1 = o.gate->c == 1;
    }
    if (o.res32) {
      FE_CHECK(!o.res && o.res32->c == y.c && o.res32->pixels() == y.pixels(), "conv: fp32 residual shape mismatch");
      p.res32 = o.res32->p; p.ldr32 = o.res32->ld;
    }
    if (o.y32) {
      FE_CHECK(o.y32->c == y.c && o.y32->pixels() == y.pixels(), "conv: fp32 output shape mismatch");
      p.y32 = o.y32->p; p.ldy32 = o.y32->ld;
    }
    p.w = (const E*)w.wh; p.y = y.p; p.ldy = y.ld;
    p.Ho = y.h; p.Wo = y.w; p.Cout = w.Cout;
    p.KH = w.KH; p.KW = w.KW; p.sh = o.sh; p.sw = o.sw; p.ph = o.ph; p.pw = o.pw; p.dh = o.dh; p.dw = o.dw;
    p.K = w.KH * w.KW * w.CinPadH; p.Kp = w.KpH; p.M = (int)y.pixels(); p.cb = w.cb;
    p.act = o.act; p.res_after_act = o.res_after_act;
    p.variant = c.force_variant;
    launch_conv_bf16(p, c.stream);
  }
  if (c.profile) {
    FE_HIP(hipEventRecord(e1, c.stream));
    FE_HIP(hipEventSynchronize(e1));
    float ms = 0.f;
    FE_HIP(hipEventElapsedTime(&ms, e0, e1));
    (void)hipEventDestroy(e0); (void)hipEventDestroy(e1);
    char nm[128];
    snprintf(nm, sizeof nm, "%s conv%dx%d s%d d%d M=%d K=%d N=%d", PrecOf<E>::value == PREC_F16 ? "f16" : "bf16", w.KH, w.KW, o.sh, o.dh, (int)y.pixels(), w.KH * w.KW * w.Cin, w.Cout);
    const double bytes = 2.0 * ((double)x.pixels() * x.c + (double)y.pixels() * y.c * (o.res ? 2 : 1) + (double)w.Cout * w.KpH);
    c.timings.push_back({nm, flops, bytes, ms});
  }
  c.flops_accum += flops;
  c.flops_half += flops;
}
void conv_forward(Ctx& c, const ConvW& w, const TensorH& x, const TensorH& y, const ConvOptsT<bf16>& o) { conv_forward_half<bf16>(c, w, x, y, o); }
void conv_forward(Ctx& c, const ConvW& w, const TensorF16& x, const TensorF16& y, const ConvOptsT<f16>& o) { conv_forward_half<f16>(c, w, x, y, o); }
// ... 384 lines not shown
```

### facet_amd/csrc/fe_common.h

```cpp
#pragma once
#include <hip/hip_runtime.h>
#include "fe_check.h"
#include <cstdint>
#include <cstdio>
#include <atomic>
#include <cstring>
#include <map>
#include <mutex>
#include <stdexcept>
#include <string>
#include <vector>

namespace fe {


#define FE_HIP(expr)                                                                      \
  do {                                                                                    \
    hipError_t _e = (expr);                                                               \
    if (_e != hipSuccess) {                                                               \
      char _b[512];                                                                       \
      snprintf(_b, sizeof _b, "%s:%d: %s -> %s", __FILE__, __LINE__, #expr,               \
               hipGetErrorString(_e));                                                    \
      throw fe::Error(_b);                                                                \
    }                                                                                     \
// ... 127 lines not shown
__device__ __forceinline__ void st4(float* p, float4 v) { *reinterpret_cast<float4*>(p) = v; }
__device__ __forceinline__ void st4(f16* p, float4 v) {
  *reinterpret_cast<uint2*>(p) = make_uint2(fe_pack2(p, v.x, v.y), fe_pack2(p, v.z, v.w));
}
__device__ __forceinline__ void st4(bf16* p, float4 v) {
  typedef __bf16 bf4 __attribute__((ext_vector_type(4)));
  bf4 o; o[0] = (bf16)v.x; o[1] = (bf16)v.y; o[2] = (bf16)v.z; o[3] = (bf16)v.w;
  *reinterpret_cast<bf4*>(p) = o;
}

class Arena {
 public:
  void init(size_t bytes) {
    release();
    FE_HIP(hipMalloc(&base_, bytes));
    cap_ = bytes;
    off_ = 0;
  }
  void release() {
    if (base_) (void)hipFree(base_);
    base_ = nullptr;
    cap_ = off_ = 0;
  }
  ~Arena() { release(); }
  void reset() { off_ = 0; }
  size_t mark() const { return off_; }
  void rewind(size_t m) { off_ = m; }
  size_t capacity() const { return cap_; }
  size_t high_water() const { return high_; }
  void* alloc(size_t bytes) {
    size_t a = (off_ + 255) & ~(size_t)255;
    FE_CHECK(a + bytes <= cap_, "arena exhausted: need %zu at %zu of %zu", bytes, a, cap_);
    off_ = a + bytes;
    if (off_ > high_) high_ = off_;
    return (char*)base_ + a;
  }
  template <class T>
  TensorT<T> tensor_t(int n, int h, int w, int c) {
    TensorT<T> t;
    t.n = n; t.h = h; t.w = w; t.c = c; t.ld = c;
    t.p = (T*)alloc(t.numel() * sizeof(T));
    return t;
  }
  Tensor tensor(int n, int h, int w, int c) { return tensor_t<float>(n, h, w, c); }
  template <class T>
  T* array(size_t count) { return (T*)alloc(count * sizeof(T)); }
 private:
  void* base_ = nullptr;
  size_t cap_ = 0, off_ = 0, high_ = 0;
};

template <class T>
struct ConvParamsT {
  const T* x; int ldx;
  const T* w;
  const float* scale;
  const float* shift;
  const float* slope;
  const T* res; int ldr;
  const T* gate; int ldg;
  T* y; int ldy;
  int N, H, W, Cin, Ho, Wo, Cout;
  int KH, KW, sh, sw, ph, pw, dh, dw;
  int K, Kp, M;
  int act;
  int res_after_act;
  int gate_c1;
  int vec_epi;
  int unit_stride;
  int ldw;
  int batch, nb1;
  long long xs1, xs2, ws1, ws2, ys1, ys2, hs1;
  int buf_ok; unsigned x_span, w_span;
  unsigned y_span, r_span, g_span;
  int variant;
  int cb;
  int pad_store;
  const float* res32; int ldr32;
  float* y32; int ldy32;
  unsigned r32_span, y32_span;
  int a_wrap;
  int split_lo_off;
  int exact_act;
};
using ConvParams = ConvParamsT<float>;
using ConvParamsH = ConvParamsT<bf16>;

struct ConvW {
  float* w = nullptr;
  float* scale = nullptr;
  float* shift = nullptr;
  float* slope = nullptr;
  int Cout = 0, Cin = 0, CinPad = 0, KH = 1, KW = 1, K = 0, Kp = 0;
  int CoutAlg = 0;
  float* wtap = nullptr;
  int wino_m = 0;
  float* wino = nullptr;
  float* wstem = nullptr;
  float* wn16 = nullptr;
  int KpT = 0;
  void* wh = nullptr;
  int hprec = 0;
  int KpH = 0, cb = 0, CinPadH = 0;
  void* wtap_h = nullptr;
  int KpTH = 0;
};

template <class T>
struct ConvOptsT {
  int sh = 1, sw = 1, ph = 0, pw = 0, dh = 1, dw = 1;
  int act = ACT_NONE;
  const TensorT<T>* res = nullptr;
  int res_after_act = 0;
  const TensorT<T>* gate = nullptr;
  const TensorT<float>* res32 = nullptr;
  const TensorT<float>* y32 = nullptr;
};
using ConvOpts = ConvOptsT<float>;

constexpr int CONV_KALIGN = 32;
constexpr int CONV_KALIGN_H = 64;

void launch_conv(const ConvParams& p, hipStream_t s);
void launch_wino_input(const Tensor& x, int th, int tw, float* V, hipStream_t s);
void launch_wino_output(const float* Mb, const Tensor& y, int th, int tw, const float* scale, const float* shift, int relu, hipStream_t s);
void launch_wino4_input(const Tensor& x, int th, int tw, float* V, hipStream_t s);
void launch_wino4_output(const float* Mb, const Tensor& y, int th, int tw, const float* scale, const float* shift, int act, const float* slope,
                         const Tensor* res, int res_after_act, hipStream_t s);
template <class TO>
bool launch_stem(const float* x, int ldx, int N, int H, int W, const float* wstem, const float* scale, const float* shift, const float* slope,
                 int Cout, int k, int stride, int act, TO* y, int ldy, int Ho, int Wo, hipStream_t s);
void launch_conv_narrow(const ConvParams& p, hipStream_t s);
void launch_conv_dma(const ConvParams& p, int tile, hipStream_t s);
void launch_conv_bf16(const ConvParamsH& p, hipStream_t s);
void launch_conv_bf16(const ConvParamsT<f16>& p, hipStream_t s);
template <class T, class Launch>
inline bool conv_split_by_images(const ConvParamsT<T>& p, Launch&& launch) {
  if (p.batch > 1 || p.N <= 1 || (long long)p.N * p.Ho * p.Wo != (long long)p.M) return false;
  const unsigned long long in_img = (unsigned long long)p.H * p.W * p.ldx * sizeof(T);
  unsigned long long out_img = (unsigned long long)p.Ho * p.Wo * (unsigned long long)(p.ldy > p.ldr ? p.ldy : p.ldr) * sizeof(T);
  const unsigned long long out32_img = (unsigned long long)p.Ho * p.Wo * (unsigned long long)(p.ldy32 > p.ldr32 ? p.ldy32 : p.ldr32) * sizeof(float);
  if ((p.y32 || p.res32) && out32_img > out_img) out_img = out32_img;
  const unsigned long long per_img = in_img > out_img ? in_img : out_img;
  constexpr unsigned long long LIMIT = 0xF0000000ull;
  if (per_img >= LIMIT) return false;
  const int ng = (int)(LIMIT / per_img);
  if (ng >= p.N) return false;
  for (int i0 = 0; i0 < p.N; i0 += ng) {
    ConvParamsT<T> q = p;
    const int n = ng < p.N - i0 ? ng : p.N - i0;
    const size_t opix = (size_t)i0 * p.Ho * p.Wo;
    q.N = n; q.M = n * p.Ho * p.Wo;
    q.x = p.x + (size_t)i0 * p.H * p.W * p.ldx;
    if (p.y) q.y = p.y + opix * p.ldy;
    if (p.y32) q.y32 = p.y32 + opix * p.ldy32;
    if (p.res32) q.res32 = p.res32 + opix * p.ldr32;
    if (p.res) q.res = p.res + opix * p.ldr;
    if (p.gate) q.gate = p.gate + opix * p.ldg;
    launch(q);
  }
  return true;
}

double conv_flops(const ConvParams& p);

void launch_u8_to_nhwc4_norm(const uint8_t* src, float* dst, size_t pixels, const float mean[3],
                             const float stdv[3], int bgr, hipStream_t s);
template <class T> void launch_nchw_to_nhwc(const float* src, T* dst, int n, int c, int h, int w, int cpad, hipStream_t s);
template <class T> void launch_nhwc_to_nchw(const T* src, int lds_, float* dst, int n, int c, int h, int w, hipStream_t s);
template <class T> void launch_maxpool(const TensorT<T>& x, const TensorT<T>& y, int k, int stride, int pad, hipStream_t s);
template <class T> void launch_bilinear(const TensorT<T>& x, const TensorT<T>& y, hipStream_t s);
template <class T> void launch_adaptive_avgpool(const TensorT<T>& x, const TensorT<T>& y, hipStream_t s);
void launch_convert(const float* x, bf16* y, size_t n, hipStream_t s);
void launch_convert(const bf16* x, float* y, size_t n, hipStream_t s);
void launch_convert(const float* x, f16* y, size_t n, hipStream_t s);
void launch_convert(const f16* x, float* y, size_t n, hipStream_t s);
void launch_splitk_reduce(const float* part, int splits, int M, int N, const float* scale, const float* shift, const float* slope, int act,
                          const float* res, int ldr, int res_after_act, float* y, int ldy, hipStream_t s);
template <class T>
void launch_tap_gather(const T* z, int ldz, int n, int h, int w, int kh, int kw, int ph, int pw, int dh, int dw,
                       int cout, const float* scale, const float* shift, int act, T* y, int ldy, int ho, int wo,
                       hipStream_t s);
void launch_attention(const float* q, int ldq, const float* k, int ldk, const float* vt, int lp, const float* bv, float* o,
                      int ldo, int B, int H, int Lq, int Lk, int dmodel, int causal, hipStream_t s);
void launch_attention(const bf16* q, int ldq, const bf16* k, int ldk, const bf16* vt, int lp, const float* bv, bf16* o,
                      int ldo, int B, int H, int Lq, int Lk, int dmodel, int causal, hipStream_t s);
void launch_attention(const f16* q, int ldq, const f16* k, int ldk, const f16* vt, int lp, const float* bv, f16* o,
                      int ldo, int B, int H, int Lq, int Lk, int dmodel, int causal, hipStream_t s);
void launch_attention_split(const f16* q, const f16* k, int ld, int lo_off, const f16* vt_hi, const f16* vt_lo, int lp, f16* o, int ldo, int o_lo_off,
                            int B, int H, int Lq, int Lk, int dmodel, hipStream_t s);
template <class TI, class TW, class TO>
void launch_gemm_skinny(const TI* x, int ldx, const TW* w, int ldw, const float* scale, const float* shift, TO* y,
                        int ldy, int M, int N, int K, int act, hipStream_t s);
void launch_sigmoid(const Tensor& x, const Tensor& y, hipStream_t s);
void launch_add(const Tensor& a, const Tensor& b, const Tensor& y, hipStream_t s);
void launch_layernorm_split(const float* x, int ldx, f16* y, int ldy, const float* g, const float* b, int rows, int d, float eps, hipStream_t s);
void launch_split_hi_lo(const float* x, f16* y, size_t rows, int cols, hipStream_t s);
// ... 63 lines not shown
```

### facet_amd/csrc/kernels_conv.hip

```cpp
#include "fe_common.h"
#include <cstdlib>

namespace fe {

typedef float f32x16 __attribute__((ext_vector_type(16)));

__device__ __forceinline__ float apply_act(float v, int act) { return fe_apply_act(v, act); }

template <int WGM, int WGN, int TM, int TN, int BK, bool FAST>
__global__ __launch_bounds__(256) void conv_igemm_kernel(ConvParams p, const int ntiles) {
  if (p.batch > 1) {
    const int b = blockIdx.y, bo = b / p.nb1, bi = b - bo * p.nb1;
    p.x += bo * p.xs2 + bi * p.xs1;
    p.w += bo * p.ws2 + bi * p.ws1;
    p.y += bo * p.ys2 + bi * p.ys1;
    if (p.shift) p.shift += bi * p.hs1;
  }
  constexpr int BM = WGM * TM * 32, BN = WGN * TN * 32;
  constexpr int S = BK + 4;
  constexpr int CH = BK / 4;
  constexpr int RPP = 256 / CH;
  constexpr int AP = (BM + RPP - 1) / RPP, BP = (BN + RPP - 1) / RPP;
  static_assert(WGM * WGN == 4, "4 waves");
  extern __shared__ __attribute__((aligned(16))) float smem[];
// ... 161 lines not shown
#pragma unroll
      for (int it = 0; it < NIT; ++it) {
        const int m = mrow0 + it * RPI;
        const int mc = m < p.M ? m : p.M - 1;
        if (p.res) rv[it] = *reinterpret_cast<const float4*>(p.res + (size_t)mc * p.ldr + colc);
        if (p.gate) {
          if (p.gate_c1) { const float g = p.gate[(size_t)mc * p.ldg]; gv[it] = make_float4(g, g, g, g); }
          else gv[it] = *reinterpret_cast<const float4*>(p.gate + (size_t)mc * p.ldg + colc);
        }
      }
#pragma unroll
      for (int it = 0; it < NIT; ++it) {
        const int m = mrow0 + it * RPI;
        float4 v = *reinterpret_cast<const float4*>(&E[(lr + it * RPI) * ES + lc]);
        v.x = v.x * sc.x + sf.x; v.y = v.y * sc.y + sf.y; v.z = v.z * sc.z + sf.z; v.w = v.w * sc.w + sf.w;
        if (p.res && !p.res_after_act) { v.x += rv[it].x; v.y += rv[it].y; v.z += rv[it].z; v.w += rv[it].w; }
        if (p.act == ACT_PRELU) {
          const float4 sl = *reinterpret_cast<const float4*>(p.slope + colc);
          v.x = v.x > 0.f ? v.x : v.x * sl.x; v.y = v.y > 0.f ? v.y : v.y * sl.y;
          v.z = v.z > 0.f ? v.z : v.z * sl.z; v.w = v.w > 0.f ? v.w : v.w * sl.w;
        } else {
          v.x = apply_act(v.x, p.act); v.y = apply_act(v.y, p.act); v.z = apply_act(v.z, p.act); v.w = apply_act(v.w, p.act);
        }
        if (p.res && p.res_after_act) { v.x += rv[it].x; v.y += rv[it].y; v.z += rv[it].z; v.w += rv[it].w; }
        if (p.gate) { v.x *= gv[it].x; v.y *= gv[it].y; v.z *= gv[it].z; v.w *= gv[it].w; }
        if (cok && m < p.M) *reinterpret_cast<float4*>(p.y + (size_t)m * p.ldy + colb) = v;
      }
    }
    return;
  }
#pragma unroll
  for (int j = 0; j < TN; ++j) {
    const int col = n0 + wn * TN * 32 + j * 32 + r;
    const bool cok = col < p.Cout;
    const float sc = (cok && p.scale) ? p.scale[col] : 1.f;
    const float sf = (cok && p.shift) ? p.shift[col] : 0.f;
#pragma unroll
    for (int i = 0; i < TM; ++i) {
#pragma unroll
      for (int e = 0; e < 16; ++e) {
        const int row = wm * TM * 32 + i * 32 + (e & 3) + 8 * (e >> 2) + 4 * h;
        const int m = m0 + row;
        if (cok && m < p.M) {
          float v = acc[i][j][e] * sc + sf;
          if (p.res && !p.res_after_act) v += p.res[(size_t)m * p.ldr + col];
          v = p.act == ACT_PRELU ? (v > 0.f ? v : v * p.slope[col]) : apply_act(v, p.act);
          if (p.res && p.res_after_act) v += p.res[(size_t)m * p.ldr + col];
          if (p.gate) v *= p.gate[(size_t)m * p.ldg + (p.gate_c1 ? 0 : col)];
          p.y[(size_t)m * p.ldy + col] = v;
        }
      }
    }
  }
}

template <int WGM, int WGN, int TM, int TN, int BK, bool FAST>
static void launch_variant(const ConvParams& p, hipStream_t s) {
  constexpr int BM = WGM * TM * 32, BN = WGN * TN * 32;
  const int mtiles = (p.M + BM - 1) / BM, ntiles = (p.Cout + BN - 1) / BN;
  const size_t lds = (size_t)2 * (BM + BN) * (BK + 4) * sizeof(float);
  auto kern = conv_igemm_kernel<WGM, WGN, TM, TN, BK, FAST>;
  static std::atomic<uint64_t> lds_set{0};
  ensure_dynamic_lds((const void*)kern, lds, lds_set);
  hipLaunchKernelGGL(kern, dim3(mtiles * ntiles, p.batch > 1 ? p.batch : 1), dim3(256), lds, s, p, ntiles);
  FE_HIP(hipGetLastError());
}

static void launch_forced(const ConvParams& q, hipStream_t s) {
  FE_CHECK(q.Cin % 16 == 0, "forced variants need Cin %% 16 == 0");
  switch (q.variant) {
    case 1: launch_variant<2, 2, 2, 2, 16, true>(q, s); break;
    case 2: launch_variant<4, 1, 2, 2, 16, true>(q, s); break;
    case 3: launch_variant<4, 1, 2, 1, 16, true>(q, s); break;
    case 4: launch_variant<2, 2, 1, 1, 16, true>(q, s); break;
    case 6: launch_variant<1, 4, 2, 2, 16, true>(q, s); break;
    case 7: launch_variant<2, 2, 2, 1, 16, true>(q, s); break;
    default: FE_CHECK(false, "unknown conv variant %d", q.variant);
  }
}

double conv_flops(const ConvParams& p) { return 2.0 * (double)p.M * p.K * p.Cout; }

void launch_conv(const ConvParams& p, hipStream_t s) {
  FE_CHECK(p.x && p.w && p.y && p.ldy >= p.Cout && p.ldx >= p.Cin, "conv: null operand or row stride below the channel count");
  FE_CHECK(p.Cin % 4 == 0 && p.ldx % 4 == 0, "conv: Cin=%d ldx=%d must be multiples of 4", p.Cin, p.ldx);
  FE_CHECK(((uintptr_t)p.x & 15) == 0 && ((uintptr_t)p.w & 15) == 0, "conv: x/w must be 16-B aligned");
  FE_CHECK(p.Kp % CONV_KALIGN == 0 && p.Kp >= p.K, "conv: bad Kp=%d K=%d", p.Kp, p.K);
  FE_CHECK(p.M > 0 && p.Cout > 0, "conv: empty problem");
  FE_CHECK((long long)p.N * p.H * p.W < (1ll << 31), "conv: too many input pixels");
  ConvParams q = p;
  if (q.ldw == 0) q.ldw = q.Kp;
  if (q.batch < 1) q.batch = 1;
  if (q.nb1 < 1) q.nb1 = 1;
  FE_CHECK(q.ldw % 4 == 0, "conv: ldw=%d must be a multiple of 4", q.ldw);
  {
    const unsigned long long xsp = (unsigned long long)p.N * p.H * p.W * (unsigned long long)p.ldx * 4;
    if (xsp >= 0xFFFFFF00ull && p.variant == 0 && conv_split_by_images(q, [&](const ConvParams& sub) { launch_conv(sub, s); })) return;
  }
  FE_CHECK(q.batch == 1 || (!q.res && !q.gate && !q.scale), "conv: batched launches take no res/gate/scale");
  auto al16 = [](const void* ptr) { return ((uintptr_t)ptr & 15) == 0; };
  q.vec_epi = (p.Cout % 4 == 0) && (p.ldy % 4 == 0) && al16(p.y) && (!p.res || (p.ldr % 4 == 0 && al16(p.res))) &&
              (!p.gate || p.gate_c1 || (p.ldg % 4 == 0 && al16(p.gate))) && (!p.scale || al16(p.scale)) &&
              (!p.shift || (al16(p.shift) && p.hs1 % 4 == 0)) && (p.batch <= 1 || (p.ys1 % 4 == 0 && p.ys2 % 4 == 0));
  const bool fast = (p.Cin % 16 == 0);
  if (q.variant > 10 && q.variant < 40) { launch_conv_dma(q, q.variant > 20 ? q.variant : q.variant - 10, s); return; }
  if (q.variant > 0) { launch_forced(q, s); return; }
  if (p.Cout <= 4 && q.batch <= 1 && !p.gate && q.variant == 0 && (p.Cin % 16 != 0 || p.KH * p.KW == 1)) { launch_conv_narrow(q, s); return; }
  static const bool no_dma = getenv("FE_NO_DMA") != nullptr;
  const unsigned long long xspan = ((unsigned long long)p.N * p.H * p.W - 1) * (unsigned long long)p.ldx * 4 + (unsigned long long)p.Cin * 4;
  const unsigned long long wspan = ((unsigned long long)p.Cout - 1) * (unsigned long long)q.ldw * 4 + (unsigned long long)p.Kp * 4;
  if (!no_dma && p.Cin % 16 == 0 && p.KH * p.KW < 64 && xspan < 0xFFFFFF00ull && wspan < 0xFFFFFF00ull) {
    struct Cand { int tile, bm, bn; double eff; };
    static const double eff7 = getenv("FE_F32_EFF7") ? atof(getenv("FE_F32_EFF7")) : 1.05;
    static const int k_short = getenv("FE_F32_KSHORT") ? atoi(getenv("FE_F32_KSHORT")) : 256;
    const Cand wide[3] = {{1, 128, 128, 1.00}, {7, 128, 64, eff7}, {4, 64, 64, 0.93}};
    static const Cand narrow[2] = {{7, 128, 64, 1.00}, {4, 64, 64, 0.95}};
    int tile = 3;
    if (p.Cout > 32) {
      const Cand* cs = p.Cout > 64 ? wide : narrow;
      const int nc = p.Cout > 64 ? 3 : 2;
      double best = 1e300;
      for (int i = 0; i < nc; ++i) {
        if (p.Cout > 64 && p.K <= k_short && cs[i].tile == 1) continue;
        const long long wgs = (long long)((p.M + cs[i].bm - 1) / cs[i].bm) * ((p.Cout + cs[i].bn - 1) / cs[i].bn) * q.batch;
        const double cost = (double)((wgs + 255) / 256) * cs[i].bm * cs[i].bn / cs[i].eff;
        if (cost < best) { best = cost; tile = cs[i].tile; }
      }
    }
    launch_conv_dma(q, tile, s);
    return;
  }
  const long long wg128 = (long long)((p.M + 127) / 128) * ((p.Cout + 127) / 128) * q.batch;
  if (p.Cout > 64) {
    if (wg128 < 384 && fast) launch_variant<2, 2, 1, 1, 16, true>(q, s);
    else if (fast) launch_variant<2, 2, 2, 2, 16, true>(q, s);
    else launch_variant<2, 2, 2, 2, 16, false>(q, s);
  } else if (p.Cout > 32) {
    if (wg128 < 192 && fast) launch_variant<2, 2, 1, 1, 16, true>(q, s);
    else if (fast) launch_variant<4, 1, 2, 2, 16, true>(q, s);
    else launch_variant<4, 1, 2, 2, 16, false>(q, s);
  } else {
    if (fast) launch_variant<4, 1, 2, 1, 16, true>(q, s);
    else launch_variant<4, 1, 2, 1, 16, false>(q, s);
  }
}

}
```

### facet_amd/csrc/kernels_conv_dma.hip

```cpp
#include "fe_common.h"
#include <cstdlib>

namespace fe {

typedef float f32x16 __attribute__((ext_vector_type(16)));
typedef float v4f __attribute__((ext_vector_type(4)));

__device__ __forceinline__ float apply_act_d(float v, int act) { return fe_apply_act(v, act); }

typedef const __attribute__((address_space(1))) void* gptr_t;
typedef __attribute__((address_space(3))) void* lptr_t;

template <int WGM, int WGN, int TM, int TN, int MODE = 0, bool ONE_TAP = false>
__global__ __launch_bounds__(256, (MODE == 1 ? 4 : (TM * TN >= 8 ? 2 : (TM * TN >= 4 ? 3 : 4)))) void conv_dma_kernel(ConvParams p, const int ntiles) {
  constexpr int BM = WGM * TM * 32, BN = WGN * TN * 32, BK = 16;
  constexpr int AI = (BM + 63) / 64, BI = (BN + 63) / 64;
  constexpr int SLAB = (BM + BN) * BK;
  static_assert(WGM * WGN == 4, "4 waves");
  extern __shared__ __attribute__((aligned(16))) float smem[];

  if (p.batch > 1) {
    const int b = blockIdx.y, bo = b / p.nb1, bi = b - bo * p.nb1;
    p.x += bo * p.xs2 + bi * p.xs1;
    p.w += bo * p.ws2 + bi * p.ws1;
    p.y += bo * p.ys2 + bi * p.ys1;
    if (p.shift) p.shift += bi * p.hs1;
  }
  const int bid = blockIdx.x, nwg = gridDim.x;
  const int q8 = nwg >> 3, rr = nwg & 7, xcd = bid & 7;
  const int swz = (xcd < rr ? xcd * (q8 + 1) : rr * (q8 + 1) + (xcd - rr) * q8) + (bid >> 3);
  const int mt = swz / ntiles, nt = swz - mt * ntiles;
  const int m0 = mt * BM, n0 = nt * BN;

  const int t = threadIdx.x;
  const int lane = t & 63, wave = __builtin_amdgcn_readfirstlane(t >> 6);
  const int wm = wave / WGN, wn = wave % WGN;
  const int r = lane & 31, h = lane >> 5;

  const int rsub = lane >> 2, slot = lane & 3;
  const int gofs = (slot ^ ((rsub >> 2) & 3)) * 4;
  unsigned aoffs[AI];
  unsigned long long amask[AI];
  const int HoWo = p.Ho * p.Wo;
  const int ntaps = p.KH * p.KW;
#pragma unroll
  for (int j = 0; j < AI; ++j) {
    const int row = 16 * (4 * j + wave) + rsub;
    const int m = m0 + row;
    const bool valid = (row < BM) && (m < p.M);
    const int mm = valid ? m : 0;
    if (ONE_TAP && p.unit_stride) {
      aoffs[j] = (unsigned)(((long long)mm * p.ldx + gofs) * 4);
      amask[j] = valid ? 1ull : 0ull;
      continue;
    }
    const int nimg = mm / HoWo;
    const int rem = mm - nimg * HoWo;
    const int oh = rem / p.Wo, ow = rem - oh * p.Wo;
    const int ih0 = oh * p.sh - p.ph, iw0 = ow * p.sw - p.pw;
    const long long pix = ((long long)nimg * p.H + ih0) * p.W + iw0;
    aoffs[j] = (unsigned)((pix * p.ldx + gofs) * 4);
    unsigned long long mk = 0;
    if (valid) {
      for (int tp = 0; tp < ntaps; ++tp) {
        const int kh = tp / p.KW, kw = tp - kh * p.KW;
        const int ih = ih0 + kh * p.dh, iw = iw0 + kw * p.dw;
        if ((unsigned)ih < (unsigned)p.H && (unsigned)iw < (unsigned)p.W) mk |= 1ull << tp;
      }
    }
    amask[j] = mk;
  }
  unsigned boffs[BI];
#pragma unroll
  for (int j = 0; j < BI; ++j) {
    const int row = 16 * (4 * j + wave) + rsub;
    int n = n0 + row;
    if (n > p.Cout - 1) n = p.Cout - 1;
    boffs[j] = (unsigned)(((size_t)n * p.ldw + gofs) * 4);
  }
  const __amdgpu_buffer_rsrc_t rsA = __builtin_amdgcn_make_buffer_rsrc(const_cast<float*>(p.x), 0, (int)p.x_span, 0x00020000);
  const __amdgpu_buffer_rsrc_t rsB = __builtin_amdgcn_make_buffer_rsrc(const_cast<float*>(p.w), 0, (int)p.w_span, 0x00020000);

  int tap = 0, kh = 0, kw = 0, ci = 0;
  const int nk = p.Kp / BK;

  float* iAb = nullptr; float* iBb = nullptr;
  int i_tb = 0, i_tbb2 = 0;
  bool i_cin_ok = true;
  auto issue_begin = [&](int kt, int buf) {
    iAb = smem + buf * SLAB;
    iBb = iAb + BM * BK;
    i_tb = ((kh * p.dh * p.W + kw * p.dw) * p.ldx + ci) * 4;
    i_tbb2 = kt * (BK * 4);
    i_cin_ok = ci < p.Cin;
  };
  auto issue_piece = [&](int q) {
    if (q < AI) {
      const int j = q;
      if (16 * (4 * j + wave) < BM) {
        const bool ok = ((amask[j] >> tap) & 1ull) && i_cin_ok;
        const unsigned off = ok ? aoffs[j] + (unsigned)i_tb : 0xFFFFFFF0u;
        __builtin_amdgcn_raw_ptr_buffer_load_lds(rsA, (lptr_t)(iAb + 256 * (4 * j + wave)), 16, (int)off, 0, 0, 0);
      }
    } else {
      const int j = q - AI;
      if (16 * (4 * j + wave) < BN)
        __builtin_amdgcn_raw_ptr_buffer_load_lds(rsB, (lptr_t)(iBb + 256 * (4 * j + wave)), 16, (int)boffs[j], i_tbb2, 0, 0);
    }
  };
  auto issue_end = [&]() {
    ++tap;
    if (++kw == p.KW) { kw = 0; ++kh; }
    if (tap == ntaps) { tap = 0; kh = 0; kw = 0; ci += BK; }
  };
  auto issue = [&](int kt, int buf) {
    issue_begin(kt, buf);
#pragma unroll
    for (int q = 0; q < AI + BI; ++q) issue_piece(q);
    issue_end();
  };

  f32x16 acc[TM][TN];
#pragma unroll
  for (int i = 0; i < TM; ++i)
#pragma unroll
    for (int j = 0; j < TN; ++j)
#pragma unroll
      for (int e = 0; e < 16; ++e) acc[i][j][e] = 0.f;

  const int sw = (r >> 2) & 3;
  const int fo0 = ((h ^ sw) << 2), fo1 = fo0 ^ 8;
  const int aoff = (wm * TM * 32 + r) * BK, boff = BM * BK + (wn * TN * 32 + r) * BK;

  constexpr int NPW_A = BM / 64;
// ... 156 lines not shown
    if constexpr ((Q) < 2 * TM * TN) {                                                                                   \
      FL_MFMA4(CUR, Q)                                                                                                   \
      FL_PIECE_AT(SLOTI, 0, Q) FL_PIECE_AT(SLOTI, 1, Q) FL_PIECE_AT(SLOTI, 2, Q) FL_PIECE_AT(SLOTI, 3, Q) FL_PIECE_AT(SLOTI, 4, Q) FL_PIECE_AT(SLOTI, 5, Q) \
    }
#define FL_SLAB(CUR, NXT, SLOTR, SLOTI)                                                                                  \
    {                                                                                                                    \
      asm volatile("s_waitcnt vmcnt(%0)" ::"i"(NPW) : "memory");                                                         \
      __builtin_amdgcn_s_barrier();                                                                                      \
      lean_begin();                                                                                                      \
      FL_READ_FRAGS(NXT, SLOTR)                                                                                          \
      __builtin_amdgcn_sched_barrier(0);                                                                                 \
      FL_STEP_Q(CUR, SLOTI, 0) FL_STEP_Q(CUR, SLOTI, 1) FL_STEP_Q(CUR, SLOTI, 2) FL_STEP_Q(CUR, SLOTI, 3)                \
      FL_STEP_Q(CUR, SLOTI, 4) FL_STEP_Q(CUR, SLOTI, 5) FL_STEP_Q(CUR, SLOTI, 6) FL_STEP_Q(CUR, SLOTI, 7)                \
      lean_end();                                                                                                        \
      asm volatile("s_waitcnt lgkmcnt(0)" ::: "memory");                                                                 \
      __builtin_amdgcn_sched_barrier(0);                                                                                 \
    }
    static_assert(NPW <= 6 && 2 * TM * TN <= 8, "lean loop: piece / MFMA slots");
#define FL_PIECE_N(SLOT, N) if constexpr ((N) < NPW) FL_PIECE(SLOT, N)
#define FL_PIECE_ALL(SLOT) FL_PIECE_N(SLOT, 0) FL_PIECE_N(SLOT, 1) FL_PIECE_N(SLOT, 2) FL_PIECE_N(SLOT, 3) FL_PIECE_N(SLOT, 4) FL_PIECE_N(SLOT, 5)
#define FL_ISSUE_ALL(SLOT) { lean_begin(); FL_PIECE_ALL(SLOT) lean_end(); }
    FL_ISSUE_ALL(0) FL_ISSUE_ALL(1) FL_ISSUE_ALL(2)
    asm volatile("s_waitcnt vmcnt(%0)" ::"i"(2 * NPW) : "memory");
    __builtin_amdgcn_s_barrier();
    FL_READ_FRAGS(0, 0)
    asm volatile("s_waitcnt lgkmcnt(0)" ::: "memory");
    __builtin_amdgcn_sched_barrier(0);
    for (int g = 0; g < nk; g += 6) {
      FL_SLAB(0, 1, 1, 0)
      FL_SLAB(1, 0, 2, 1)
      if (g + 2 < nk) {
        FL_SLAB(0, 1, 0, 2)
        FL_SLAB(1, 0, 1, 0)
      }
      if (g + 4 < nk) {
        FL_SLAB(0, 1, 2, 1)
        FL_SLAB(1, 0, 0, 2)
      }
    }
    asm volatile("s_waitcnt vmcnt(0)" ::: "memory");
#undef FL_SLAB
#undef FL_STEP_Q
#undef FL_PIECE_AT
#undef FL_MFMA4
#undef FL_READ_FRAGS
#undef FL_READ1
#undef FL_PIECE
#undef FL_ISSUE_ALL
#undef FL_PIECE_N
#undef FL_PIECE_ALL
  } else if constexpr (MODE == 1) {
    issue(0, 0);
    wait_vm(0);
    __builtin_amdgcn_s_barrier();
    for (int kt = 0; kt < nk; ++kt) {
      if (kt + 1 < nk) issue(kt + 1, (kt + 1) & 1);
      FE_READ_FRAGS(0, kt & 1)
      asm volatile("s_waitcnt lgkmcnt(0)" ::: "memory");
      __builtin_amdgcn_sched_barrier(0);
      FE_MFMA_BURST(0)
      wait_vm(0);
      __builtin_amdgcn_s_barrier();
    }
  } else {
    issue(0, 0);
    if (nk > 1) issue(1, 1);
    if (nk > 2) issue(2, 2);
    wait_vm(nk > 2 ? 2 * npw : (nk > 1 ? npw : 0));
    __builtin_amdgcn_s_barrier();
    FE_READ_FRAGS(0, 0)
    asm volatile("s_waitcnt lgkmcnt(0)" ::: "memory");
    __builtin_amdgcn_sched_barrier(0);
    for (int kt = 0; kt < nk; kt += 2) {
      FE_STEP(0, 1, kt)
      if (kt + 1 < nk) FE_STEP(1, 0, kt + 1)
    }
  }
#undef FE_STEP
#undef FE_MFMA_BURST_ISSUE
#undef FE_MFMA_BURST
#undef FE_READ_FRAGS
  __syncthreads();

  if constexpr (TN == 1) {
    if (p.vec_epi) {
      constexpr int WC = TN * 32, ES = WC + 4, LPR = WC / 4, RPI = 64 / LPR, NIT = 32 / RPI;
      float* E = smem + wave * 32 * ES;
      const int lr = lane / LPR, lc = (lane % LPR) * 4;
      const int colb = n0 + wn * WC + lc;
      const bool cok = colb < p.Cout;
      const int colc = cok ? colb : 0;
      float4 sc = make_float4(1.f, 1.f, 1.f, 1.f), sf = make_float4(0.f, 0.f, 0.f, 0.f);
      if (p.scale) sc = *reinterpret_cast<const float4*>(p.scale + colc);
      if (p.shift) sf = *reinterpret_cast<const float4*>(p.shift + colc);
      constexpr bool RES_AHEAD = (TM * NIT <= 8);
      float4 rall[RES_AHEAD ? TM * NIT : 1];
      if constexpr (RES_AHEAD) {
        if (p.res) {
  #pragma unroll
          for (int i = 0; i < TM; ++i)
  #pragma unroll
            for (int it = 0; it < NIT; ++it) {
              const int m = m0 + wm * TM * 32 + i * 32 + lr + it * RPI;
              const int mc = m < p.M ? m : p.M - 1;
              rall[i * NIT + it] = *reinterpret_cast<const float4*>(p.res + (size_t)mc * p.ldr + colc);
            }
        }
      }
  #pragma unroll
      for (int i = 0; i < TM; ++i) {
  #pragma unroll
        for (int j = 0; j < TN; ++j)
  #pragma unroll
          for (int e = 0; e < 16; ++e) E[((e & 3) + 8 * (e >> 2) + 4 * h) * ES + j * 32 + r] = acc[i][j][e];
        const int mrow0 = m0 + wm * TM * 32 + i * 32 + lr;
        float4 rv[NIT], gv[NIT];
  #pragma unroll
        for (int it = 0; it < NIT; ++it) {
          const int m = mrow0 + it * RPI;
          const int mc = m < p.M ? m : p.M - 1;
          if constexpr (RES_AHEAD) { if (p.res) rv[it] = rall[i * NIT + it]; }
          else if (p.res) rv[it] = *reinterpret_cast<const float4*>(p.res + (size_t)mc * p.ldr + colc);
          if (p.gate) {
            if (p.gate_c1) { const float g = p.gate[(size_t)mc * p.ldg]; gv[it] = make_float4(g, g, g, g); }
            else gv[it] = *reinterpret_cast<const float4*>(p.gate + (size_t)mc * p.ldg + colc);
          }
        }
  #pragma unroll
        for (int it = 0; it < NIT; ++it) {
          const int m = mrow0 + it * RPI;
          float4 v = *reinterpret_cast<const float4*>(&E[(lr + it * RPI) * ES + lc]);
          v.x = v.x * sc.x + sf.x; v.y = v.y * sc.y + sf.y; v.z = v.z * sc.z + sf.z; v.w = v.w * sc.w + sf.w;
          if (p.res && !p.res_after_act) { v.x += rv[it].x; v.y += rv[it].y; v.z += rv[it].z; v.w += rv[it].w; }
          if constexpr (MODE == 2) {
            const float4 sl = *reinterpret_cast<const float4*>(p.slope + colc);
            v.x = v.x > 0.f ? v.x : v.x * sl.x; v.y = v.y > 0.f ? v.y : v.y * sl.y;
            v.z = v.z > 0.f ? v.z : v.z * sl.z; v.w = v.w > 0.f ? v.w : v.w * sl.w;
          } else {
            v.x = apply_act_d(v.x, p.act); v.y = apply_act_d(v.y, p.act); v.z = apply_act_d(v.z, p.act); v.w = apply_act_d(v.w, p.act);
          }
          if (p.res && p.res_after_act) { v.x += rv[it].x; v.y += rv[it].y; v.z += rv[it].z; v.w += rv[it].w; }
          if (p.gate) { v.x *= gv[it].x; v.y *= gv[it].y; v.z *= gv[it].z; v.w *= gv[it].w; }
          if (cok && m < p.M) *reinterpret_cast<float4*>(p.y + (size_t)m * p.ldy + colb) = v;
        }
      }
      return;
    }
  #pragma unroll
    for (int j = 0; j < TN; ++j) {
      const int col = n0 + wn * TN * 32 + j * 32 + r;
      const bool cok = col < p.Cout;
      const float sc = (cok && p.scale) ? p.scale[col] : 1.f;
      const float sf = (cok && p.shift) ? p.shift[col] : 0.f;
  #pragma unroll
      for (int i = 0; i < TM; ++i) {
  #pragma unroll
        for (int e = 0; e < 16; ++e) {
          const int row = wm * TM * 32 + i * 32 + (e & 3) + 8 * (e >> 2) + 4 * h;
          const int m = m0 + row;
          if (cok && m < p.M) {
            float v = acc[i][j][e] * sc + sf;
            if (p.res && !p.res_after_act) v += p.res[(size_t)m * p.ldr + col];
            if constexpr (MODE == 2) v = v > 0.f ? v : v * p.slope[col];
            else v = apply_act_d(v, p.act);
            if (p.res && p.res_after_act) v += p.res[(size_t)m * p.ldr + col];
            if (p.gate) v *= p.gate[(size_t)m * p.ldg + (p.gate_c1 ? 0 : col)];
// ... 62 lines not shown
  #pragma unroll
        for (int e = 0; e < 4; ++e) v[e] = 1.f / (1.f + __expf(-v[e]));
      } else if (act == ACT_SOFTPLUS) {
  #pragma unroll 1
        for (int e = 0; e < 4; ++e) v[e] = v[e] > 20.f ? v[e] : log1pf(expf(v[e]));
      }
  #pragma unroll
      for (int e = 0; e < 4; ++e) {
        float x = v[e];
        if (p.res && p.res_after_act) x += rf[e];
        if (p.gate) x *= gf[e];
        v[e] = x;
      }
      if (cok && m < p.M) {
        float* yp = p.y + (size_t)m * p.ldy + colb;
        if (vec) {
          *reinterpret_cast<float4*>(yp) = make_float4(v[0], v[1], v[2], v[3]);
        } else {
  #pragma unroll
          for (int e = 0; e < 4; ++e)
            if (colb + e < p.Cout) yp[e] = v[e];
        }
      }
    };
    constexpr bool AHEAD = (TM * NIT <= 8);
    float4 rall[AHEAD ? TM * NIT : 1];
    if constexpr (AHEAD) {
  #pragma unroll
      for (int i = 0; i < TM; ++i)
  #pragma unroll
        for (int it = 0; it < NIT; ++it) rall[i * NIT + it] = fetch_res(row_of(i, it));
    }
  #pragma unroll
    for (int i = 0; i < TM; ++i) {
  #pragma unroll
      for (int j = 0; j < TN; ++j)
  #pragma unroll
        for (int e = 0; e < 16; ++e) E[((e & 3) + 8 * (e >> 2) + 4 * h) * ES + j * 32 + r] = acc[i][j][e];
      if constexpr (AHEAD) {
        float4 ev[NIT];
  #pragma unroll
        for (int it = 0; it < NIT; ++it) ev[it] = read_row(lr + it * RPI);
  #pragma unroll
        for (int it = 0; it < NIT; ++it) finish_row(row_of(i, it), ev[it], rall[i * NIT + it], fetch_gate(row_of(i, it)));
      } else {
        float4 rn = fetch_res(row_of(i, 0)), gn = fetch_gate(row_of(i, 0));
  #pragma unroll 1
        for (int it = 0; it < NIT; ++it) {
          const float4 ru = rn, gu = gn;
          if (it + 1 < NIT) { rn = fetch_res(row_of(i, it + 1)); gn = fetch_gate(row_of(i, it + 1)); }
          finish_row(row_of(i, it), read_row(lr + it * RPI), ru, gu);
        }
      }
    }
  
  }
}

template <int WGM, int WGN, int TM, int TN, int MODE = 0, bool ONE_TAP = false>
static void launch_dma_variant(const ConvParams& p, hipStream_t s) {
  constexpr int BM = WGM * TM * 32, BN = WGN * TN * 32;
  const int mtiles = (p.M + BM - 1) / BM, ntiles = (p.Cout + BN - 1) / BN;
  constexpr size_t main_lds = (size_t)(MODE == 1 ? 2 : 3) * (BM + BN) * 16 * sizeof(float) + (BN == 32 ? 4096 : 0);
  constexpr size_t epi_lds = (size_t)4 * 32 * (TN * 32 + 4) * sizeof(float);
  constexpr size_t lds = main_lds > epi_lds ? main_lds : epi_lds;
  auto kern = conv_dma_kernel<WGM, WGN, TM, TN, MODE, ONE_TAP>;
  static std::atomic<uint64_t> lds_set{0};
  ensure_dynamic_lds((const void*)kern, lds, lds_set);
  hipLaunchKernelGGL(kern, dim3(mtiles * ntiles, p.batch > 1 ? p.batch : 1), dim3(256), lds, s, p, ntiles);
  FE_HIP(hipGetLastError());
}

void launch_conv_dma(const ConvParams& p0, int tile, hipStream_t s) {
  FE_CHECK(p0.Cin % 16 == 0 && p0.KH * p0.KW < 64, "conv_dma: needs Cin %% 16 == 0 and < 64 taps");
  ConvParams p = p0;
  const unsigned long long xs = ((unsigned long long)p.N * p.H * p.W - 1) * (unsigned long long)p.ldx * 4 + (unsigned long long)p.Cin * 4;
  const unsigned long long ws = ((unsigned long long)p.Cout - 1) * (unsigned long long)p.ldw * 4 + (unsigned long long)p.Kp * 4;
  static const bool no_buf = getenv("FE_NO_BUF") != nullptr;
  p.buf_ok = !no_buf && xs < 0xFFFFFF00ull && ws < 0xFFFFFF00ull;
  FE_CHECK(p.buf_ok, "conv_dma: operand spans exceed 32-bit buffer addressing (caller must use the register-staged kernel)");
  p.x_span = (unsigned)xs; p.w_span = (unsigned)ws;
  p.unit_stride = (p.KH == 1 && p.KW == 1 && p.sh == 1 && p.sw == 1 && p.ph == 0 && p.pw == 0 && p.Ho == p.H && p.Wo == p.W &&
                   (long long)p.N * p.H * p.W == (long long)p.M) ? 1 : 0;
  if (p.act == ACT_PRELU) {
    FE_CHECK(p.slope, "conv_dma: PReLU without slopes");
    switch (tile) {
      case 3: launch_dma_variant<4, 1, 2, 1, 2>(p, s); break;
      case 4: launch_dma_variant<2, 2, 1, 1, 2>(p, s); break;
      case 2: case 22: case 7: launch_dma_variant<2, 2, 2, 1, 2>(p, s); break;
      default: launch_dma_variant<2, 2, 2, 2, 2>(p, s); break;
    }
    return;
  }
  if (p.KH * p.KW == 1 && p.Cin % 32 == 0 && p.Kp == p.Cin) {
    switch (tile) {
      case 1: launch_dma_variant<2, 2, 2, 2, 0, true>(p, s); return;
      case 7: launch_dma_variant<2, 2, 2, 1, 0, true>(p, s); return;
      case 4: launch_dma_variant<2, 2, 1, 1, 0, true>(p, s); return;
      default: break;
    }
  }
  switch (tile) {
    case 1: launch_dma_variant<2, 2, 2, 2>(p, s); break;
    case 21: launch_dma_variant<2, 2, 2, 2, 1>(p, s); break;
    case 22: launch_dma_variant<4, 1, 2, 2, 1>(p, s); break;
    case 2: launch_dma_variant<4, 1, 2, 2>(p, s); break;
    case 3: launch_dma_variant<4, 1, 2, 1>(p, s); break;
    case 4: launch_dma_variant<2, 2, 1, 1>(p, s); break;
    case 7: launch_dma_variant<2, 2, 2, 1>(p, s); break;
    case 8: launch_dma_variant<2, 2, 4, 2>(p, s); break;
    case 9: launch_dma_variant<2, 2, 2, 4>(p, s); break;
    default: FE_CHECK(false, "conv_dma: unknown tile %d", tile);
  }
}

}
```

### facet_amd/csrc/model_topiq.hip

```cpp
#include "engine.h"
#include <algorithm>
#include <cmath>

namespace fe {

static EncLayerW build_enc(DeviceWeights& dw, const WeightStore& ws, const std::string& p, int heads) {
  EncLayerW e;
  e.attn = build_mha(dw, ws, p + ".self_attn", heads);
  e.lin1 = build_linear(dw, ws, p + ".linear1", true);
  e.lin2 = build_linear(dw, ws, p + ".linear2", true);
  e.n1 = build_ln(dw, ws, p + ".norm1");
  e.n2 = build_ln(dw, ws, p + ".norm2");
  return e;
}

static DecLayerW build_dec(DeviceWeights& dw, const WeightStore& ws, const std::string& p, int heads) {
  DecLayerW d;
  d.cross = build_mha(dw, ws, p + ".multihead_attn", heads);
  d.lin1 = build_linear(dw, ws, p + ".linear1", true);
  d.lin2 = build_linear(dw, ws, p + ".linear2", true);
  d.n1 = build_ln(dw, ws, p + ".norm1");
  d.n2 = build_ln(dw, ws, p + ".norm2");
  d.n3 = build_ln(dw, ws, p + ".norm3");
  return d;
// ... 62 lines not shown
  const float scale = (float)in / (float)out;
  const float real = scale * ((float)o + 0.5f) - 0.5f;
  const float fl = std::floor(real);
  const float t = real - fl;
  const int i0 = (int)fl;
  const float A = -0.75f;
  auto c1 = [&](float x) { return ((A + 2.f) * x - (A + 3.f)) * x * x + 1.f; };
  auto c2 = [&](float x) { return ((A * x - 5.f * A) * x + 8.f * A) * x - 4.f * A; };
  wt[0] = c2(t + 1.f); wt[1] = c1(t); wt[2] = c1(1.f - t); wt[3] = c2(2.f - t);
  for (int k = 0; k < 4; ++k) {
    int j = i0 - 1 + k;
    idx[k] = j < 0 ? 0 : (j > in - 1 ? in - 1 : j);
  }
}

static float* topiq_pos(TopiqModel& m, int th, int tw) {
  auto key = std::make_pair(th, tw);
  auto it = m.pos.find(key);
  if (it != m.pos.end()) return it->second;
  std::vector<float> hy((size_t)th * 128), wx((size_t)tw * 128);
  int idx[4]; float wt[4];
  for (int y = 0; y < th; ++y) {
    cubic_taps(th, 32, y, idx, wt);
    for (int c = 0; c < 128; ++c) {
      float acc = 0.f;
      for (int k = 0; k < 4; ++k) acc += wt[k] * m.h_emb[(size_t)c * 32 + idx[k]];
      hy[(size_t)y * 128 + c] = acc;
    }
  }
  for (int x = 0; x < tw; ++x) {
    cubic_taps(tw, 32, x, idx, wt);
    for (int c = 0; c < 128; ++c) {
      float acc = 0.f;
      for (int k = 0; k < 4; ++k) acc += wt[k] * m.w_emb[(size_t)c * 32 + idx[k]];
      wx[(size_t)x * 128 + c] = acc;
    }
  }
  std::vector<float> pos((size_t)th * tw * 256);
  for (int y = 0; y < th; ++y)
    for (int x = 0; x < tw; ++x) {
      float* d = &pos[((size_t)y * tw + x) * 256];
      for (int c = 0; c < 128; ++c) { d[c] = hy[(size_t)y * 128 + c]; d[128 + c] = wx[(size_t)x * 128 + c]; }
    }
  float* dev = m.dw.upload(pos);
  m.pos[key] = dev;
  return dev;
}

template <class T>
static void ln(Ctx& c, const LayerNormW& l, const T* x, T* y, int rows) {
  launch_layernorm(x, l.d, y, l.d, l.g, l.b, rows, l.d, l.eps, c.stream);
}

template <class T>
static void enc_forward(Ctx& c, const EncLayerW& e, T* x, T* y, int B, int L) {
  const int d = e.n1.d, rows = B * L, ff = e.lin1.Cout;
  const size_t mark = c.arena.mark();
  T* n = c.arena.array<T>((size_t)rows * d);
  T* a = c.arena.array<T>((size_t)rows * d);
  T* hbuf = c.arena.array<T>((size_t)rows * ff);
  ln(c, e.n1, x, n, rows);
  mha_forward<T>(c, e.attn, n, d, n, d, B, L, L, x, d, a, d);
  ln(c, e.n2, a, n, rows);
  linear_forward(c, e.lin1, n, d, rows, hbuf, ff, ACT_GELU);
  linear_forward(c, e.lin2, hbuf, ff, rows, y, d, ACT_NONE, a, d);
  c.arena.rewind(mark);
}

template <class T>
static void dec_forward(Ctx& c, const DecLayerW& w, T* tgt, const T* memory, int B, int Lq, int Lk) {
  const int d = w.n1.d, ff = w.lin1.Cout;
  const size_t mark = c.arena.mark();
  T* mem = c.arena.array<T>((size_t)B * Lk * d);
  T* t2 = c.arena.array<T>((size_t)B * Lq * d);
  T* a = c.arena.array<T>((size_t)B * Lq * d);
  T* hbuf = c.arena.array<T>((size_t)B * Lq * ff);
  ln(c, w.n2, memory, mem, B * Lk);
  ln(c, w.n1, (const T*)tgt, t2, B * Lq);
  mha_forward<T>(c, w.cross, t2, d, mem, d, B, Lq, Lk, tgt, d, a, d);
  ln(c, w.n3, (const T*)a, t2, B * Lq);
  linear_forward(c, w.lin1, t2, d, B * Lq, hbuf, ff, ACT_GELU);
  linear_forward(c, w.lin2, hbuf, ff, B * Lq, tgt, d, ACT_NONE, a, d);
  c.arena.rewind(mark);
}

template <class T>
void topiq_head_forward(Ctx& c, TopiqModel& m, const std::vector<TensorT<T>>& feats, float* scores_dev) {
  FE_CHECK(m.has_head && feats.size() == 5, "topiq head: not built / bad pyramid");
  const int B = feats[0].n;
  const int th = feats[4].h, tw = feats[4].w, L = th * tw, d = 256;
  const float* pos = topiq_pos(m, th, tw);
  T* tok[5];
  for (int i = 0; i < 5; ++i) tok[i] = c.arena.array<T>((size_t)B * L * d);
  for (int i = 4; i >= 0; --i) {
    const size_t mark = c.arena.mark();
    const TensorT<T>& f = feats[i];
    const GatedConvW& g = m.gate[i];
    if constexpr (sizeof(T) == 2) {
      const bool no_fused = getenv("FE_NO_FUSED_GATE") != nullptr;
      if (g.fused && !no_fused && f.c == 64 && f.h == 16 * th && f.w == 16 * tw && f.ld % 8 == 0) {
        TensorT<T> pooled = c.arena.tensor_t<T>(B, th, tw, 64);
        const double px = (double)f.pixels(), flops = 2.0 * px * (64.0 * 64 + 576.0 * 64 + 576.0 + 64.0 * 64);
        hipEvent_t e0 = nullptr, e1 = nullptr;
        if (c.profile) { FE_HIP(hipEventCreate(&e0)); FE_HIP(hipEventCreate(&e1)); FE_HIP(hipEventRecord(e0, c.stream)); }
        launch_topiq_gate64(f, pooled, g.fused, g.fused_bias, m.wblk_act, m.gate_act, c.stream);
        if (c.profile) {
          FE_HIP(hipEventRecord(e1, c.stream)); FE_HIP(hipEventSynchronize(e1));
          float ms = 0.f;
          FE_HIP(hipEventElapsedTime(&ms, e0, e1));
          (void)hipEventDestroy(e0); (void)hipEventDestroy(e1);
          char nm[128];
          snprintf(nm, sizeof nm, "%s fused gate64 + pool16 M=%d", PrecOf<T>::value == PREC_F16 ? "f16" : "bf16", (int)f.pixels());
          c.timings.push_back({nm, flops, 2.0 * px * 64, ms});
        }
        c.flops_accum += flops; c.flops_half += flops;
        TensorT<T> t = mat_view(tok[i], B * L, d, d);
        t.n = B; t.h = th; t.w = tw;
        ConvOptsT<T> od; od.act = ACT_GELU;
        conv_forward(c, m.dim_reduce[i], pooled, t, od);
        launch_add_rows_bcast(tok[i], d, pos, B * L, L, d, c.stream);
        enc_forward(c, m.sa[i], tok[i], tok[i], B, L);
        c.arena.rewind(mark);
        continue;
      }
    }
    ConvOptsT<T> o0; o0.act = m.wblk_act;
    TensorT<T> wa = conv_new(c, g.w0, f, o0);
    ConvOptsT<T> o2; o2.act = m.wblk_act; o2.ph = o2.pw = 1;
    TensorT<T> wb;
    bool tiled = false;
    if constexpr (sizeof(T) == 2) {
      if (g.w2_frag && wa.c == 64 && wa.ld == 64 && !g.w2.scale && wa.pixels() >= 131072 && !getenv("FE_NO_FUSED_C64")) {
        wb = c.arena.tensor_t<T>(wa.n, wa.h, wa.w, 64);
        const double flops = 2.0 * (double)wa.pixels() * 576.0 * 64;
        hipEvent_t e0 = nullptr, e1 = nullptr;
        if (c.profile) { FE_HIP(hipEventCreate(&e0)); FE_HIP(hipEventCreate(&e1)); FE_HIP(hipEventRecord(e0, c.stream)); }
        launch_conv3x3_c64(wa, wb, (const TensorT<T>*)nullptr, g.w2_frag, nullptr, nullptr, g.w2.shift, nullptr, nullptr, m.wblk_act, c.stream);
        if (c.profile) {
          FE_HIP(hipEventRecord(e1, c.stream)); FE_HIP(hipEventSynchronize(e1));
          float ms = 0.f;
          FE_HIP(hipEventElapsedTime(&ms, e0, e1));
          (void)hipEventDestroy(e0); (void)hipEventDestroy(e1);
          char nm[128];
          snprintf(nm, sizeof nm, "%s halo-tiled conv3x3 64->64 M=%d", PrecOf<T>::value == PREC_F16 ? "f16" : "bf16", (int)wa.pixels());
          c.timings.push_back({nm, flops, 2.0 * (double)wa.pixels() * 128, ms});
        }
        c.flops_accum += flops; c.flops_half += flops;
        tiled = true;
      }
    }
    if (!tiled) wb = conv_new(c, g.w2, wa, o2);
    ConvOptsT<T> o4; o4.act = ACT_SIGMOID; o4.ph = o4.pw = 1;
    TensorT<T> wc = conv_new(c, g.w4, wb, o4);
    ConvOptsT<T> og; og.act = m.gate_act; og.gate = &wc;
    TensorT<T> gated = conv_new(c, g.split_x1, f, og);
    if (gated.h > th && gated.w > tw) {
      TensorT<T> pooled = c.arena.tensor_t<T>(B, th, tw, gated.c);
      launch_adaptive_avgpool(gated, pooled, c.stream);
      gated = pooled;
    }
    FE_CHECK(gated.h == th && gated.w == tw, "topiq head: level %d is %dx%d, expected %dx%d", i, gated.h, gated.w, th, tw);
    TensorT<T> t = mat_view(tok[i], B * L, d, d);
    t.n = B; t.h = th; t.w = tw;
    ConvOptsT<T> od; od.act = ACT_GELU;
    conv_forward(c, m.dim_reduce[i], gated, t, od);
    launch_add_rows_bcast(tok[i], d, pos, B * L, L, d, c.stream);
    enc_forward(c, m.sa[i], tok[i], tok[i], B, L);
    c.arena.rewind(mark);
  }
  T* query = tok[4];
  for (int i = 0; i < 4; ++i) dec_forward(c, m.cross[i], query, (const T*)tok[3 - i], B, L, L);
  enc_forward(c, m.pool, query, query, B, L);
  TensorT<T> fin; fin.p = query; fin.n = B; fin.h = 1; fin.w = L; fin.c = d; fin.ld = d;
  TensorT<T> mean = c.arena.tensor_t<T>(B, 1, 1, d);
  launch_adaptive_avgpool(fin, mean, c.stream);
  float* a = c.arena.array<float>((size_t)B * d);
  float* b = c.arena.array<float>((size_t)B * d);
  const float* mean_f = to_f32(c, mean.p, (size_t)B * d);
  launch_layernorm(mean_f, d, a, d, m.s_ln0.g, m.s_ln0.b, B, d, m.s_ln0.eps, c.stream);
  linear_forward(c, m.s_l1, (const float*)a, d, B, b, d, ACT_GELU);
  launch_layernorm((const float*)b, d, a, d, m.s_ln3.g, m.s_ln3.b, B, d, m.s_ln3.eps, c.stream);
  linear_forward(c, m.s_l4, (const float*)a, d, B, b, d, ACT_GELU);
  linear_forward(c, m.s_l6, (const float*)b, d, B, scores_dev, 1, ACT_NONE);
}
template void topiq_head_forward<float>(Ctx&, TopiqModel&, const std::vector<Tensor>&, float*);
template void topiq_head_forward<bf16>(Ctx&, TopiqModel&, const std::vector<TensorH>&, float*);
template void topiq_head_forward<f16>(Ctx&, TopiqModel&, const std::vector<TensorF16>&, float*);

}
```

### include/facet_engine.h

```cpp
#ifndef FACET_ENGINE_H
#define FACET_ENGINE_H

#include <stddef.h>
#include <stdint.h>

#ifdef __cplusplus
extern "C" {
#endif

typedef struct fe_ctx fe_ctx;

enum fe_status {
  FE_OK = 0,
  FE_ERR_INVALID = -1,
  FE_ERR_RUNTIME = -2,
  FE_ERR_NOT_LOADED = -3,
  FE_ERR_CAPACITY = -4
};

enum fe_model {
  FE_MODEL_TOPIQ = 0,
  FE_MODEL_CLIP = 1,
  FE_MODEL_SAMP = 2,
  FE_MODEL_U2NETP = 3,
  FE_MODEL_AESTHETIC = 4,
  FE_MODEL_VLM = 5
};

enum fe_act { FE_ACT_NONE = 0, FE_ACT_RELU = 1, FE_ACT_GELU = 2, FE_ACT_SIGMOID = 3, FE_ACT_SOFTPLUS = 5  };

int fe_create(int device, size_t arena_bytes, fe_ctx** out);
void fe_destroy(fe_ctx* ctx);
const char* fe_last_error(fe_ctx* ctx);
const char* fe_version(void);
int fe_sync(fe_ctx* ctx);
int fe_set_microbatch(fe_ctx* ctx, int n);

enum fe_precision { FE_PRECISION_F32 = 0, FE_PRECISION_BF16 = 1, FE_PRECISION_F16 = 2, FE_PRECISION_RES32 = 16, FE_PRECISION_SPLIT3 = 32 };
int fe_set_precision(fe_ctx* ctx, int precision);
int fe_model_precision(fe_ctx* ctx, int model);

int fe_vlm_configure(fe_ctx* ctx, int n_heads, int n_kv_heads, int head_dim, float rope_theta, float rms_eps, const int* mrope_section);
int fe_vlm_vision_configure(fe_ctx* ctx, int n_heads, const int* fullatt_block_indexes, int n_fullatt);
int fe_vlm_encode_images(fe_ctx* ctx, const float* pixel_values, int n_patches, const int32_t* patch_pos_hw, const int32_t* window_index,
                         const int32_t* cu_window_seqlens, int n_windows, const int32_t* cu_seqlens, int n_images, float* embeds);
int fe_vlm_prefill_images(fe_ctx* ctx, const int32_t* tokens, const int32_t* position_ids, int n_seq, int len, int max_seq, const int32_t* image_rows,
                          int n_image_rows, int32_t* next_tokens, float* logits);
int fe_vlm_dims(fe_ctx* ctx, int* dims8);
int fe_vlm_prefill(fe_ctx* ctx, const int32_t* tokens, const int32_t* position_ids, int n_seq, int len, int max_seq, int32_t* next_tokens,
                   float* logits);
int fe_vlm_decode_step(fe_ctx* ctx, const int32_t* tokens, const int32_t* position_ids, int n_seq, int32_t* next_tokens, float* logits);
int fe_vlm_generate(fe_ctx* ctx, const int32_t* tokens, const int32_t* position_ids, int n_seq, int n_steps, int32_t* out_tokens);
int fe_vlm_generate_scored(fe_ctx* ctx, const int32_t* tokens, const int32_t* position_ids, int n_seq, int n_steps, int32_t* out_tokens,
                           float* out_logprobs);
int fe_vlm_last_logprobs(fe_ctx* ctx, float* out);
int fe_vlm_preprocess_rgb(fe_ctx* ctx, const uint8_t* rgb, int n_images, const int32_t* sizes, const float* mean, const float* stdv, float* pixel_values);
int fe_vlm_encode_preprocessed(fe_ctx* ctx, const int32_t* patch_pos_hw, const int32_t* window_index, const int32_t* cu_window_seqlens, int n_windows,
                               const int32_t* cu_seqlens, int n_images, float* embeds);
int fe_vlm_prefill_images_padded(fe_ctx* ctx, const int32_t* tokens, const int32_t* position_ids, int n_seq, int len, int max_seq, const int32_t* pad,
                                 const int32_t* image_rows, int n_image_rows, int32_t* next_tokens, float* logits);

int fe_vlm_vision_dims(fe_ctx* ctx, int* dims4);
int fe_vlm3_configure(fe_ctx* ctx, int n_heads, int n_kv_heads, int head_dim, float rope_theta, float rms_eps, const int* mrope_section, int vis_heads,
                      const int* deepstack_indexes, int n_deepstack);
int fe_vlm3_encode_images(fe_ctx* ctx, const float* pixel_values, int n_patches, const int32_t* patch_pos_hw, const int32_t* interp_idx, const float* interp_w,
                          const int32_t* cu_seqlens, int n_seg, float* embeds, float* deepstack);

int fe_vlm2_configure(fe_ctx* ctx, int n_heads, int n_kv_heads, int head_dim, float rope_theta, float rms_eps, const int* mrope_section, int vis_heads);
int fe_vlm2_encode_images(fe_ctx* ctx, const float* pixel_values, int n_patches, const int32_t* patch_pos_hw, const int32_t* cu_seqlens, int n_seg, float* embeds);
int fe_vlm_generate_until(fe_ctx* ctx, const int32_t* tokens, const int32_t* position_ids, int n_seq, int max_steps, const int32_t* eos_ids, int n_eos, int poll,
                          int32_t* out_tokens, float* out_logprobs, int* steps_run);

int fe_dev_alloc(fe_ctx* ctx, size_t bytes, void** d_out);
int fe_dev_free(fe_ctx* ctx, void* d_ptr);
int fe_memcpy_h2d(fe_ctx* ctx, void* d_dst, const void* src, size_t bytes);
int fe_memcpy_d2h(fe_ctx* ctx, void* dst, const void* d_src, size_t bytes);

int fe_timer_start(fe_ctx* ctx);
int fe_timer_stop(fe_ctx* ctx, float* ms_out);
int fe_profile_enable(fe_ctx* ctx, int on);
int fe_profile_count(fe_ctx* ctx);
int fe_profile_get(fe_ctx* ctx, int i, char* name, int name_cap, double* flops, double* bytes, float* ms);
int fe_flops_reset(fe_ctx* ctx);
int fe_flops_get(fe_ctx* ctx, double* flops);
int fe_flops_get_executed(fe_ctx* ctx, double* flops);
int fe_flops_get_half(fe_ctx* ctx, double* flops);

int fe_weights_begin(fe_ctx* ctx, int model);
int fe_weights_set(fe_ctx* ctx, int model, const char* name, const float* data, const int64_t* shape, int ndim);
int fe_weights_commit(fe_ctx* ctx, int model);
int fe_model_unload(fe_ctx* ctx, int model);
int fe_model_loaded(fe_ctx* ctx, int model);

int fe_op_conv2d(fe_ctx* ctx, const float* x, int n, int c, int h, int w, const float* weight, int cout, int kh,
                 int kw, const float* scale, const float* shift, const float* res, int res_after_act, int stride,
                 int pad, int dil, int act, float* y);
int fe_op_topiq_gate64(fe_ctx* ctx, const float* x, int n, int h, int w, const float* w0, const float* b0, const float* w2,
                       const float* b2, const float* w4, float b4, const float* wx, const float* bx, int wblk_act,
                       int gate_act, float* y);
int fe_op_conv3x3_c64(fe_ctx* ctx, const float* x, int n, int h, int w, const float* w2, const float* scale2,
                      const float* shift2, int act2, const float* w3, const float* scale3, const float* shift3,
                      const float* res, float* y);
int fe_op_maxpool2d(fe_ctx* ctx, const float* x, int n, int c, int h, int w, int k, int stride, int pad,
                    int ceil_mode, float* y);
int fe_op_bilinear(fe_ctx* ctx, const float* x, int n, int c, int h, int w, int ho, int wo, float* y);
int fe_op_adaptive_avgpool(fe_ctx* ctx, const float* x, int n, int c, int h, int w, int ho, int wo, float* y);
int fe_op_layernorm(fe_ctx* ctx, const float* x, int rows, int d, const float* g, const float* b, float eps, float* y);
int fe_op_vlm_select(fe_ctx* ctx, const float* logits, int rows, int vocab, int32_t* ids, float* logprobs);

int fe_set_conv_variant(fe_ctx* ctx, int variant);
int fe_bench_conv(fe_ctx* ctx, int n, int h, int w, int cin, int cout, int k, int stride, int pad, int with_res, int act,
                  int variant, int iters, float* ms_out);

int fe_topiq_configure(fe_ctx* ctx, int gate_act, int weight_blk_act);
int fe_topiq_f32_below(fe_ctx* ctx, long long pixels);
int fe_topiq_feature_shape(int h, int w, int level, int dims[3]);
int fe_topiq_features(fe_ctx* ctx, const uint8_t* rgb, int n, int h, int w, int on_device, int level, float* out);
int fe_topiq_score(fe_ctx* ctx, const uint8_t* rgb, int n, int h, int w, int on_device, float* scores);

int fe_u2netp_saliency(fe_ctx* ctx, const float* x, int n, int h, int w, float* sal_out);
int fe_samp_forward(fe_ctx* ctx, const float* x, int n, float* pattern_weights, float* attributes, float* score_dist,
                    float* sal_out);

int fe_clip_encode_image(fe_ctx* ctx, const float* x, int n, int on_device, float* features, float* emb_norm,
                         float* aesthetic_raw);

int fe_aesthetic_score(fe_ctx* ctx, const float* feats, int n, float* aesthetic_raw);

enum fe_filter { FE_LANCZOS = 1, FE_BILINEAR = 2, FE_BICUBIC = 3 };
int fe_resize_u8(fe_ctx* ctx, const uint8_t* src, int n, int h, int w, int oh, int ow, int filter, int on_device,
                 uint8_t* dst);

int fe_resize_u8_box(fe_ctx* ctx, const uint8_t* src, int n, int h, int w, int oh, int ow, int filter, const float* box, int on_device,
                     uint8_t* dst);
int fe_reduce_u8(fe_ctx* ctx, const uint8_t* src, int n, int h, int w, int fx, int fy, const int32_t* box, int on_device, uint8_t* dst);

size_t fe_jpeg_bound(int h, int w);
int fe_jpeg_encode(fe_ctx* ctx, const uint8_t* img, int n, int h, int w, int bgr, int on_device, int quality, uint8_t* out, size_t cap,
                   int32_t* lengths);
int fe_thumbnail_jpeg(fe_ctx* ctx, const uint8_t* img, int n, int h, int w, int bgr, int on_device, int oh, int ow, int fx, int fy,
                      const int32_t* reduce_box, const float* resize_box, int tall, int quality, uint8_t* out, size_t cap, int32_t* lengths);

#define FE_FACE_THUMB_FUSED_SIDE 128
#define FE_FACE_THUMB_MAX_SIDE 8192
int fe_face_thumbnails(fe_ctx* ctx, const uint8_t* bgr, int n, int h, int w, int on_device, int m, const int32_t* img_index,
                       const int32_t* crops, const int32_t* out_sizes, int quality, uint8_t* out, size_t cap, int32_t* lengths);

#define FE_JPEG_OK 0
#define FE_JPEG_PROGRESSIVE 1
#define FE_JPEG_ARITHMETIC 2
#define FE_JPEG_PRECISION 3
#define FE_JPEG_COMPONENTS 4
#define FE_JPEG_ADOBE_RGB 5
#define FE_JPEG_SAMPLING 6
#define FE_JPEG_MULTISCAN 7
#define FE_JPEG_OTHER 8
#define FE_JPEG_BAD_MARKER (-1)
#define FE_JPEG_BAD_HUFFMAN (-2)
#define FE_JPEG_PREMATURE_END (-3)
#define FE_JPEG_BAD_RESTART (-4)
#define FE_JPEG_BAD_DIMENSIONS (-5)
#define FE_JPEG_BAD_COEFFICIENT (-6)
typedef struct { int32_t width, height, components, hsamp, vsamp, restart_interval, orientation, status; } fe_jpeg_info;
int fe_jpeg_probe(const uint8_t* data, size_t len, fe_jpeg_info* info);
int fe_jpeg_decode(fe_ctx* ctx, const uint8_t* const* data, const size_t* len, int n, int h, int w, int bgr, int apply_orientation,
                   int dst_on_device, uint8_t* dst, int32_t* status);
typedef struct { int32_t width, height, components, hsamp, vsamp, restart_interval, orientation, status, progressive, scans; } fe_jpeg_info_ex;
int fe_jpeg_probe_ex(const uint8_t* data, size_t len, int flags, fe_jpeg_info_ex* info);
int fe_jpeg_decode_ex(fe_ctx* ctx, const uint8_t* const* data, const size_t* len, int n, int h, int w, int bgr, int apply_orientation,
                      int dst_on_device, int flags, uint8_t* dst, int32_t* status);
int fe_jpeg_scaled_size(int h, int w, int scale, int32_t* scaled_h, int32_t* scaled_w);
int fe_jpeg_decode_scaled(fe_ctx* ctx, const uint8_t* const* data, const size_t* len, int n, int h, int w, int scale, int bgr,
                          int apply_orientation, int dst_on_device, int flags, uint8_t* dst, int32_t* status);
int fe_jpeg_thumbnail(fe_ctx* ctx, const uint8_t* const* data, const size_t* len, int n, int h, int w, int scale, int flags, int oh, int ow,
                      int fx, int fy, const int32_t* reduce_box, const float* resize_box, int tall, int quality, uint8_t* out, size_t cap,
                      int32_t* lengths, int32_t* status);

int fe_clip_encode_images(fe_ctx* ctx, const uint8_t* rgb, int n, int h, int w, int on_device, float* features,
                          float* emb_norm, float* aesthetic_raw);
int fe_samp_score_images(fe_ctx* ctx, const uint8_t* img, int n, int h, int w, int bgr, int on_device,
                         float* pattern_weights, float* attributes, float* score_dist);
int fe_clip_encode_text(fe_ctx* ctx, const int32_t* tokens, int n, int ctx_len, float* features);
// ... 94 lines not shown
```

Measured before the change: 228.9.

## Fuse f32 TOPIQ gate conv with avg-pool and 3x3 conv with tap conv

Adds an f32 path for the TOPIQ gated-conv head. The 1x1 gate conv gets a pooling epilogue in the DMA conv kernel, so the full-resolution gated map is never written and re-read. The 3x3 64-channel conv now writes per-tap products of the following sigmoid conv, and a gather kernel finishes that conv, which avoids materialising the 64-channel intermediate. It also adds a standalone C API for testing, with env switches to turn each fusion off; the new epilogues bring alignment and shape preconditions that fall back to the unfused path.

```diff
diff --git a/facet_amd/_lib.py b/facet_amd/_lib.py
--- a/facet_amd/_lib.py
+++ b/facet_amd/_lib.py
@@ -77,6 +77,8 @@
                                C.c_int, _f32p, _f32p, _f32p, C.c_int, C.c_int, C.c_int, C.c_int, C.c_int, _f32p]),
     "fe_op_topiq_gate64": (C.c_int, [C.c_void_p, _f32p, C.c_int, C.c_int, C.c_int, _f32p, _f32p, _f32p, _f32p, _f32p, C.c_float,
                                      _f32p, _f32p, C.c_int, C.c_int, _f32p]),
+    "fe_op_topiq_gate_f32": (C.c_int, [C.c_void_p, _f32p, C.c_int, C.c_int, C.c_int, C.c_int, _f32p, _f32p, _f32p, _f32p, _f32p, C.c_float,
+                                       _f32p, _f32p, C.c_int, C.c_int, C.c_int, C.c_int, _f32p]),
     "fe_op_conv3x3_c64": (C.c_int, [C.c_void_p, _f32p, C.c_int, C.c_int, C.c_int, _f32p, _f32p, _f32p, C.c_int, _f32p, _f32p, _f32p,
                                     _f32p, _f32p]),
     "fe_op_maxpool2d": (C.c_int, [C.c_void_p, _f32p, C.c_int, C.c_int, C.c_int, C.c_int, C.c_int, C.c_int,
@@ -456,6 +458,16 @@
                                              arrs[5][1], arrs[6][1], ACT[wblk_act], ACT[gate_act], y.ctypes.data_as(_f32p)))
         return y
 
+    def topiq_gate_f32(self, x, w0, b0, w2, b2, w4, b4, wx, bx, out_hw, wblk_act="gelu", gate_act="gelu"):
+        x, xp = _f32(x)
+        n, c, h, w = x.shape
+        ho, wo = out_hw
+        arrs = [_f32(a) for a in (w0, b0, w2, b2, w4, wx, bx)]
+        y = np.empty((n, c, ho, wo), np.float32)
+        self._ck(self.lib.fe_op_topiq_gate_f32(self.h, xp, n, c, h, w, arrs[0][1], arrs[1][1], arrs[2][1], arrs[3][1], arrs[4][1], C.c_float(float(b4)),
+                                               arrs[5][1], arrs[6][1], ACT[wblk_act], ACT[gate_act], int(ho), int(wo), y.ctypes.data_as(_f32p)))
+        return y
+
     def conv3x3_c64(self, x, w2, scale2=None, shift2=None, act2="relu", w3=None, scale3=None, shift3=None, res=None):
         x, xp = _f32(x)
         n, c, h, w = x.shape
diff --git a/facet_amd/csrc/capi.hip b/facet_amd/csrc/capi.hip
--- a/facet_amd/csrc/capi.hip
+++ b/facet_amd/csrc/capi.hip
@@ -608,6 +608,39 @@
     download_nchw(C, yt, 64, y);
   };
   if (C.precision == PREC_BF16) run((bf16*)nullptr); else run((f16*)nullptr);
+  FE_API_END(ctx)
+}
+
+int fe_op_topiq_gate_f32(fe_ctx* ctx, const float* x, int n, int c, int h, int w, const float* w0, const float* b0, const float* w2, const float* b2,
+                         const float* w4, float b4, const float* wx, const float* bx, int wblk_act, int gate_act, int ho, int wo, float* y) {
+  FE_API_BEGIN(ctx)
+  Ctx& C = ctx->c;
+  FE_CHECK(x && w0 && b0 && w2 && b2 && w4 && wx && bx && y && n > 0 && c > 0 && c % 4 == 0 && h > 0 && w > 0 && ho > 0 && wo > 0 && ho <= h && wo <= w,
+           "bad topiq_gate_f32 arguments");
+  FE_CHECK(C.precision == PREC_F32, "fe_op_topiq_gate_f32: the fp32 route only");
+  C.arena.reset();
+  DeviceWeights dw;
+  dw.prec = PREC_F32;
+  auto host = [](const float* p, std::vector<int64_t> shape) {
+    HostTensor t;
+    size_t cnt = 1;
+    for (int64_t d : shape) cnt *= (size_t)d;
+    t.shape = std::move(shape);
+    t.data.assign(p, p + cnt);
+    return t;
+  };
+  const HostTensor W0 = host(w0, {64, c}), B0 = host(b0, {64}), Wx = host(wx, {c, c}), Bx = host(bx, {c});
+  const HostTensor W2 = host(w2, {64, 64, 3, 3}), W4 = host(w4, {1, 64, 3, 3});
+  const std::vector<float> s2(b2, b2 + 64), s4(1, b4);
+  GatedConvW g;
+  g.split_x1 = build_linear_rows(dw, Wx, &Bx, 0, c);
+  g.w0 = build_linear_rows(dw, W0, &B0, 0, 64);
+  g.w2 = pack_conv(dw, W2, nullptr, &s2);
+  g.w4 = pack_conv(dw, W4, nullptr, &s4);
+  Tensor xt = upload_nchw(C, x, n, c, h, w, c);
+  Tensor yt = topiq_gate_forward_f32(C, g, xt, ho, wo, wblk_act, gate_act);
+  FE_CHECK(yt.h == ho && yt.w == wo, "fe_op_topiq_gate_f32: the %dx%d map does not pool to %dx%d", h, w, ho, wo);
+  download_nchw(C, yt, c, y);
   FE_API_END(ctx)
 }
 
diff --git a/facet_amd/csrc/engine.h b/facet_amd/csrc/engine.h
--- a/facet_amd/csrc/engine.h
+++ b/facet_amd/csrc/engine.h
@@ -123,6 +123,8 @@
 void conv_forward(Ctx& c, const ConvW& w, const Tensor& x, const Tensor& y, const ConvOpts& o);
 void conv_forward(Ctx& c, const ConvW& w, const TensorH& x, const TensorH& y, const ConvOptsT<bf16>& o);
 void conv_forward(Ctx& c, const ConvW& w, const TensorF16& x, const TensorF16& y, const ConvOptsT<f16>& o);
+bool conv_tap_fusable(const Ctx& c, const ConvW& w, const ConvOpts& o, const ConvW& wn, const ConvOpts& on, const Tensor& x);
+void conv_tap_forward(Ctx& c, const ConvW& w, const ConvOpts& o, const ConvW& wn, const ConvOpts& on, const Tensor& x, const Tensor& y);
 template <class T>
 TensorT<T> conv_new(Ctx& c, const ConvW& w, const TensorT<T>& x, const ConvOptsT<T>& o);
 template <class T>
@@ -252,6 +254,8 @@
                             const float* Wx, const float* Bx);
 template <class E>
 void launch_topiq_gate64(const TensorT<E>& x, const TensorT<E>& out, const void* frag, const float* bias, int wblk_act, int gate_act, hipStream_t s);
+
+Tensor topiq_gate_forward_f32(Ctx& c, const GatedConvW& g, const Tensor& f, int th, int tw, int wblk_act, int gate_act);
 
 struct TopiqModel {
   DeviceWeights dw;
diff --git a/facet_amd/csrc/engine.hip b/facet_amd/csrc/engine.hip
--- a/facet_amd/csrc/engine.hip
+++ b/facet_amd/csrc/engine.hip
@@ -231,6 +231,22 @@
   return l;
 }
 
+struct LaunchTimer {
+  Ctx& c;
+  hipEvent_t e0 = nullptr, e1 = nullptr;
+  explicit LaunchTimer(Ctx& ctx) : c(ctx) {
+    if (c.profile) { FE_HIP(hipEventCreate(&e0)); FE_HIP(hipEventCreate(&e1)); FE_HIP(hipEventRecord(e0, c.stream)); }
+  }
+  void end(const char* name, double flops, double bytes) {
+    if (!c.profile) return;
+    FE_HIP(hipEventRecord(e1, c.stream)); FE_HIP(hipEventSynchronize(e1));
+    float ms = 0.f;
+    FE_HIP(hipEventElapsedTime(&ms, e0, e1));
+    (void)hipEventDestroy(e0); (void)hipEventDestroy(e1);
+    c.timings.push_back({name, flops, bytes, ms});
+  }
+};
+
 void conv_forward(Ctx& c, const ConvW& w, const Tensor& x, const Tensor& y, const ConvOpts& o) {
   FE_CHECK(x.c == w.CinPad, "conv: input channels %d != packed Cin %d", x.c, w.CinPad);
   FE_CHECK(y.c == w.Cout && y.n == x.n, "conv: output view mismatch (c=%d Cout=%d)", y.c, w.Cout);
@@ -257,6 +273,40 @@
   FE_CHECK(y.pixels() < (1ull << 31), "conv: M too large");
   p.act = o.act; p.res_after_act = o.res_after_act;
   p.variant = c.force_variant;
+  if (o.pool) {
+    const Tensor& pl = *o.pool;
+    FE_CHECK(pl.p && pl.n == x.n && pl.c == w.Cout && pl.h > 0 && pl.w > 0 && pl.h <= y.h && pl.w <= y.w, "conv: pooled output view mismatch");
+    const int sd = (y.h % pl.h == 0 && y.w % pl.w == 0 && y.h / pl.h == y.w / pl.w) ? y.h / pl.h : 0;
+    const int ls = sd == 2 ? 1 : sd == 4 ? 2 : sd == 8 ? 3 : 0;
+    auto al16 = [](const void* q) { return ((uintptr_t)q & 15) == 0; };
+    const unsigned long long xspan = (unsigned long long)x.pixels() * (unsigned long long)x.ld * 4;
+    const bool fuse = ls && w.w && w.KH == 1 && w.KW == 1 && o.sh == 1 && o.sw == 1 && o.ph == 0 && o.pw == 0 && y.h == x.h && y.w == x.w &&
+                      w.CinPad % 32 == 0 && w.Kp == w.CinPad && w.Cout % 64 == 0 && !o.res && o.act != ACT_PRELU && (!o.gate || o.gate->c == 1) &&
+                      p.variant == 0 && pl.ld % 4 == 0 && al16(pl.p) && x.ld % 4 == 0 && al16(x.p) && (!w.scale || al16(w.scale)) &&
+                      (!w.shift || al16(w.shift)) && xspan < 0xFFFFFF00ull && !getenv("FE_NO_DMA") && !getenv("FE_NO_BUF");
+    const size_t mark = c.arena.mark();
+    if (!fuse) {
+      ConvOpts of = o;
+      of.pool = nullptr;
+      Tensor full = y;
+      if (!full.p) full = c.arena.tensor(y.n, y.h, y.w, y.c);
+      conv_forward(c, w, x, full, of);
+      launch_adaptive_avgpool(full, pl, c.stream);
+      c.arena.rewind(mark);
+      return;
+    }
+    p.y = pl.p; p.ldy = pl.ld;
+    p.pool_ls = ls; p.pool_th = pl.h; p.pool_tw = pl.w;
+    LaunchTimer tm(c);
+    launch_conv(p, c.stream);
+    char nm[128];
+    snprintf(nm, sizeof nm, "conv1x1 + pool%d M=%d K=%d N=%d", sd, p.M, p.K, p.Cout);
+    tm.end(nm, 2.0 * p.M * (double)w.Cin * (w.CoutAlg ? w.CoutAlg : p.Cout),
+           4.0 * ((double)x.pixels() * x.c + (double)pl.pixels() * pl.c + (double)w.Cout * w.K));
+    c.arena.rewind(mark);
+    c.flops_accum += 2.0 * p.M * (double)(w.KH * w.KW * w.Cin) * (w.CoutAlg ? w.CoutAlg : p.Cout);
+    return;
+  }
   if (w.wtap && o.act != ACT_PRELU && o.sh == 1 && o.sw == 1 && !o.res && !o.gate && p.variant == 0 && y.h == x.h && y.w == x.w) {
     const int T = w.KH * w.KW * w.Cout, Tp = (T + 3) & ~3;
     const size_t mark = c.arena.mark();
@@ -385,6 +435,42 @@
     launch();
   }
   c.flops_accum += 2.0 * p.M * (double)(w.KH * w.KW * w.Cin) * (w.CoutAlg ? w.CoutAlg : p.Cout);
+}
+
+bool conv_tap_fusable(const Ctx& c, const ConvW& w, const ConvOpts& o, const ConvW& wn, const ConvOpts& on, const Tensor& x) {
+  const int T = wn.KH * wn.KW * wn.Cout;
+  auto al16 = [](const void* q) { return ((uintptr_t)q & 15) == 0; };
+  const unsigned long long xspan = (unsigned long long)x.pixels() * (unsigned long long)x.ld * 4;
+  return w.w && w.Cout == 64 && w.KH == 3 && w.KW == 3 && w.CinPad % 16 == 0 && x.c == w.CinPad && o.sh == 1 && o.sw == 1 && o.ph == 1 && o.pw == 1 &&
+         o.dh == 1 && o.dw == 1 && !o.res && !o.gate && !o.pool && o.act != ACT_PRELU && wn.wtap && wn.CinPad == 64 && T <= 12 && wn.KpT >= 64 &&
+         wn.KpT % 4 == 0 && on.sh == 1 && on.sw == 1 && on.ph == wn.KH / 2 && on.pw == wn.KW / 2 && on.dh == 1 && on.dw == 1 && !on.res && !on.gate &&
+         !on.pool && on.act != ACT_PRELU && c.force_variant == 0 && x.ld % 4 == 0 && al16(x.p) && (!w.scale || al16(w.scale)) &&
+         (!w.shift || al16(w.shift)) && xspan < 0xFFFFFF00ull && x.pixels() < (1ull << 31) && !getenv("FE_NO_DMA") && !getenv("FE_NO_BUF");
+}
+
+void conv_tap_forward(Ctx& c, const ConvW& w, const ConvOpts& o, const ConvW& wn, const ConvOpts& on, const Tensor& x, const Tensor& y) {
+  FE_CHECK(conv_tap_fusable(c, w, o, wn, on, x), "conv_tap: layer pair not fusable");
+  FE_CHECK(y.c == wn.Cout && y.n == x.n && y.h == x.h && y.w == x.w, "conv_tap: output view mismatch");
+  const int T = wn.KH * wn.KW * wn.Cout, Tp = (T + 3) & ~3;
+  const size_t mark = c.arena.mark();
+  Tensor z = c.arena.tensor(x.n, x.h, x.w, Tp);
+  ConvParams p{};
+  p.x = x.p; p.ldx = x.ld; p.w = w.w; p.scale = w.scale; p.shift = w.shift; p.y = z.p; p.ldy = Tp;
+  p.N = x.n; p.H = x.h; p.W = x.w; p.Cin = w.CinPad; p.Ho = x.h; p.Wo = x.w; p.Cout = w.Cout;
+  p.KH = w.KH; p.KW = w.KW; p.sh = p.sw = 1; p.ph = o.ph; p.pw = o.pw; p.dh = p.dw = 1;
+  p.K = w.K; p.Kp = w.Kp; p.M = (int)x.pixels(); p.act = o.act;
+  p.tapw = wn.wtap; p.tap_t = T; p.tap_ld = wn.KpT;
+  LaunchTimer tm(c);
+  launch_conv(p, c.stream);
+  char nm[128];
+  snprintf(nm, sizeof nm, "conv3x3 + %d taps M=%d K=%d N=%d", T, p.M, p.K, p.Cout);
+  tm.end(nm, 2.0 * p.M * (double)(w.KH * w.KW * w.Cin) * p.Cout + 2.0 * p.M * 64.0 * T,
+         4.0 * ((double)x.pixels() * x.c + (double)x.pixels() * Tp + (double)w.Cout * w.K));
+  launch_tap_gather(z.p, Tp, x.n, x.h, x.w, wn.KH, wn.KW, on.ph, on.pw, on.dh, on.dw, wn.Cout, wn.scale, wn.shift, on.act, y.p, y.ld, y.h, y.w,
+                    c.stream);
+  c.arena.rewind(mark);
+  c.flops_accum += 2.0 * p.M * (double)(w.KH * w.KW * w.Cin) * (w.CoutAlg ? w.CoutAlg : p.Cout);
+  c.flops_accum += 2.0 * p.M * (double)(wn.KH * wn.KW * wn.Cin) * (wn.CoutAlg ? wn.CoutAlg : wn.Cout);
 }
 
 template <class E>
diff --git a/facet_amd/csrc/fe_common.h b/facet_amd/csrc/fe_common.h
--- a/facet_amd/csrc/fe_common.h
+++ b/facet_amd/csrc/fe_common.h
@@ -233,6 +233,9 @@
   int a_wrap;
   int split_lo_off;
   int exact_act;
+  int pool_ls, pool_th, pool_tw;
+  const float* tapw;
+  int tap_t, tap_ld;
 };
 using ConvParams = ConvParamsT<float>;
 using ConvParamsH = ConvParamsT<bf16>;
@@ -264,6 +267,7 @@
   const TensorT<T>* res = nullptr;
   int res_after_act = 0;
   const TensorT<T>* gate = nullptr;
+  const TensorT<T>* pool = nullptr;
   const TensorT<float>* res32 = nullptr;
   const TensorT<float>* y32 = nullptr;
 };
diff --git a/facet_amd/csrc/kernels_conv.hip b/facet_amd/csrc/kernels_conv.hip
--- a/facet_amd/csrc/kernels_conv.hip
+++ b/facet_amd/csrc/kernels_conv.hip
@@ -267,7 +267,7 @@
 double conv_flops(const ConvParams& p) { return 2.0 * (double)p.M * p.K * p.Cout; }
 
 void launch_conv(const ConvParams& p, hipStream_t s) {
-  FE_CHECK(p.x && p.w && p.y && p.ldy >= p.Cout && p.ldx >= p.Cin, "conv: null operand or row stride below the channel count");
+  FE_CHECK(p.x && p.w && p.y && (p.ldy >= p.Cout || p.tapw) && p.ldx >= p.Cin, "conv: null operand or row stride below the channel count");
   FE_CHECK(p.Cin % 4 == 0 && p.ldx % 4 == 0, "conv: Cin=%d ldx=%d must be multiples of 4", p.Cin, p.ldx);
   FE_CHECK(((uintptr_t)p.x & 15) == 0 && ((uintptr_t)p.w & 15) == 0, "conv: x/w must be 16-B aligned");
   FE_CHECK(p.Kp % CONV_KALIGN == 0 && p.Kp >= p.K, "conv: bad Kp=%d K=%d", p.Kp, p.K);
@@ -280,7 +280,7 @@
   FE_CHECK(q.ldw % 4 == 0, "conv: ldw=%d must be a multiple of 4", q.ldw);
   {
     const unsigned long long xsp = (unsigned long long)p.N * p.H * p.W * (unsigned long long)p.ldx * 4;
-    if (xsp >= 0xFFFFFF00ull && p.variant == 0 && conv_split_by_images(q, [&](const ConvParams& sub) { launch_conv(sub, s); })) return;
+    if (xsp >= 0xFFFFFF00ull && p.variant == 0 && !p.pool_ls && !p.tapw && conv_split_by_images(q, [&](const ConvParams& sub) { launch_conv(sub, s); })) return;
   }
   FE_CHECK(q.batch == 1 || (!q.res && !q.gate && !q.scale), "conv: batched launches take no res/gate/scale");
   auto al16 = [](const void* ptr) { return ((uintptr_t)ptr & 15) == 0; };
@@ -288,6 +288,7 @@
               (!p.gate || p.gate_c1 || (p.ldg % 4 == 0 && al16(p.gate))) && (!p.scale || al16(p.scale)) &&
               (!p.shift || (al16(p.shift) && p.hs1 % 4 == 0)) && (p.batch <= 1 || (p.ys1 % 4 == 0 && p.ys2 % 4 == 0));
   const bool fast = (p.Cin % 16 == 0);
+  if (q.pool_ls || q.tapw) { launch_conv_dma(q, 7, s); return; }
   if (q.variant > 10 && q.variant < 40) { launch_conv_dma(q, q.variant > 20 ? q.variant : q.variant - 10, s); return; }
   if (q.variant > 0) { launch_forced(q, s); return; }
   if (p.Cout <= 4 && q.batch <= 1 && !p.gate && q.variant == 0 && (p.Cin % 16 != 0 || p.KH * p.KW == 1)) { launch_conv_narrow(q, s); return; }
diff --git a/facet_amd/csrc/kernels_conv_dma.hip b/facet_amd/csrc/kernels_conv_dma.hip
--- a/facet_amd/csrc/kernels_conv_dma.hip
+++ b/facet_amd/csrc/kernels_conv_dma.hip
@@ -39,6 +39,11 @@
 
   const int rsub = lane >> 2, slot = lane & 3;
   const int gofs = (slot ^ ((rsub >> 2) & 3)) * 4;
+  auto pool_win = [&](int wq) -> int {
+    const int wx = wq % p.pool_tw, t2 = wq / p.pool_tw, wy = t2 % p.pool_th, img = t2 / p.pool_th;
+    return (img * p.H + (wy << p.pool_ls)) * p.W + (wx << p.pool_ls);
+  };
+  auto pool_in = [&](int q) -> int { return (q >> p.pool_ls) * p.W + (q & ((1 << p.pool_ls) - 1)); };
   unsigned aoffs[AI];
   unsigned long long amask[AI];
   const int HoWo = p.Ho * p.Wo;
@@ -50,6 +55,10 @@
     const bool valid = (row < BM) && (m < p.M);
     const int mm = valid ? m : 0;
     if (ONE_TAP && p.unit_stride) {
+      if constexpr (MODE == 3) {
+        const long long pix = pool_win(mm >> (2 * p.pool_ls)) + pool_in(mm & ((1 << (2 * p.pool_ls)) - 1));
+        aoffs[j] = (unsigned)((pix * p.ldx + gofs) * 4);
+      } else
       aoffs[j] = (unsigned)(((long long)mm * p.ldx + gofs) * 4);
       amask[j] = valid ? 1ull : 0ull;
       continue;
@@ -372,6 +381,98 @@
 #undef FE_READ_FRAGS
   __syncthreads();
 
+  if constexpr (MODE == 3) {
+    constexpr int ES = 36;
+    static_assert(4 * 64 * ES <= 3 * SLAB, "pooling epilogue: staging exceeds the ring");
+    float* E = smem + wave * 64 * ES;
+    const int lr = lane >> 3, lc = (lane & 7) * 4;
+    const int colb = n0 + wn * 32 + lc;
+    const int ls = p.pool_ls, l2 = 2 * ls, qmask = (1 << l2) - 1;
+    const int mw = m0 + wm * 64;
+    if (mw >= p.M) return;
+    float4 sc = make_float4(1.f, 1.f, 1.f, 1.f), sf = make_float4(0.f, 0.f, 0.f, 0.f);
+    if (p.scale) sc = *reinterpret_cast<const float4*>(p.scale + colb);
+    if (p.shift) sf = *reinterpret_cast<const float4*>(p.shift + colb);
+    const int wbase = ls >= 3 ? pool_win(mw >> l2) : 0;
+    float gv[8];
+  #pragma unroll
+    for (int k = 0; k < 8; ++k) {
+      const int m = mw + k * 8 + lr;
+      const int mc = m < p.M ? m : p.M - 1;
+      const int pix = (ls >= 3 ? wbase : pool_win(mc >> l2)) + pool_in(mc & qmask);
+      gv[k] = p.gate ? p.gate[(size_t)pix * p.ldg] : 1.f;
+    }
+  #pragma unroll
+    for (int i = 0; i < TM; ++i)
+  #pragma unroll
+      for (int e = 0; e < 16; ++e) E[(i * 32 + (e & 3) + 8 * (e >> 2) + 4 * h) * ES + r] = acc[i][0][e];
+  #pragma unroll
+    for (int k = 0; k < 8; ++k) {
+      float4* ep = reinterpret_cast<float4*>(&E[(lr + k * 8) * ES + lc]);
+      float4 u = *ep;
+      u.x = apply_act_d(u.x * sc.x + sf.x, p.act); u.y = apply_act_d(u.y * sc.y + sf.y, p.act);
+      u.z = apply_act_d(u.z * sc.z + sf.z, p.act); u.w = apply_act_d(u.w * sc.w + sf.w, p.act);
+      if (p.gate) { u.x *= gv[k]; u.y *= gv[k]; u.z *= gv[k]; u.w *= gv[k]; }
+      *ep = u;
+    }
+    const int g = 1 << l2;
+    const float cnt = (float)g;
+    for (int gi = h; gi * g < 64; gi += 2) {
+      const int mfirst = mw + gi * g;
+      if (mfirst >= p.M) break;
+      const float* ep = E + gi * g * ES + r;
+      float a = 0.f;
+      for (int q = 0; q < g; ++q) a += ep[q * ES];
+      p.y[(size_t)(mfirst >> l2) * p.ldy + n0 + wn * 32 + r] = a / cnt;
+    }
+    return;
+  } else if constexpr (MODE == 4) {
+    constexpr int ES = 68;
+    static_assert(BM * ES <= 3 * SLAB, "tap epilogue: staging exceeds the ring");
+    float* E = smem + wm * 64 * ES;
+    const int lr = lane >> 3, lc = (lane & 7) * 4;
+    const int colb = wn * 32 + lc;
+    float4 sc = make_float4(1.f, 1.f, 1.f, 1.f), sf = make_float4(0.f, 0.f, 0.f, 0.f);
+    if (p.scale) sc = *reinterpret_cast<const float4*>(p.scale + colb);
+    if (p.shift) sf = *reinterpret_cast<const float4*>(p.shift + colb);
+  #pragma unroll
+    for (int i = 0; i < TM; ++i)
+  #pragma unroll
+      for (int e = 0; e < 16; ++e) E[(i * 32 + (e & 3) + 8 * (e >> 2) + 4 * h) * ES + wn * 32 + r] = acc[i][0][e];
+  #pragma unroll
+    for (int k = 0; k < 8; ++k) {
+      float4* ep = reinterpret_cast<float4*>(&E[(lr + k * 8) * ES + colb]);
+      float4 u = *ep;
+      u.x = apply_act_d(u.x * sc.x + sf.x, p.act); u.y = apply_act_d(u.y * sc.y + sf.y, p.act);
+      u.z = apply_act_d(u.z * sc.z + sf.z, p.act); u.w = apply_act_d(u.w * sc.w + sf.w, p.act);
+      *ep = u;
+    }
+    __syncthreads();
+    f32x16 d;
+  #pragma unroll
+    for (int e = 0; e < 16; ++e) d[e] = 0.f;
+    const float* arow = E + (wn * 32 + r) * ES + 4 * h;
+    const float* brow = p.tapw + (size_t)(r < p.tap_t ? r : 0) * p.tap_ld + 4 * h;
+    const bool bok = r < p.tap_t;
+  #pragma unroll
+    for (int ks = 0; ks < 8; ++ks) {
+      const float4 a = *reinterpret_cast<const float4*>(arow + 8 * ks);
+      float4 b = *reinterpret_cast<const float4*>(brow + 8 * ks);
+      if (!bok) b = make_float4(0.f, 0.f, 0.f, 0.f);
+      d = __builtin_amdgcn_mfma_f32_32x32x2f32(a.x, b.x, d, 0, 0, 0);
+      d = __builtin_amdgcn_mfma_f32_32x32x2f32(a.y, b.y, d, 0, 0, 0);
+      d = __builtin_amdgcn_mfma_f32_32x32x2f32(a.z, b.z, d, 0, 0, 0);
+      d = __builtin_amdgcn_mfma_f32_32x32x2f32(a.w, b.w, d, 0, 0, 0);
+    }
+    if (r < p.ldy) {
+  #pragma unroll
+      for (int e = 0; e < 16; ++e) {
+        const int m = m0 + wm * 64 + wn * 32 + (e & 3) + 8 * (e >> 2) + 4 * h;
+        if (m < p.M) p.y[(size_t)m * p.ldy + r] = d[e];
+      }
+    }
+    return;
+  } else
   if constexpr (TN == 1) {
     if (p.vec_epi) {
       constexpr int WC = TN * 32, ES = WC + 4, LPR = WC / 4, RPI = 64 / LPR, NIT = 32 / RPI;
@@ -600,6 +701,21 @@
   p.x_span = (unsigned)xs; p.w_span = (unsigned)ws;
   p.unit_stride = (p.KH == 1 && p.KW == 1 && p.sh == 1 && p.sw == 1 && p.ph == 0 && p.pw == 0 && p.Ho == p.H && p.Wo == p.W &&
                    (long long)p.N * p.H * p.W == (long long)p.M) ? 1 : 0;
+  if (p.pool_ls) {
+    const int g = 1 << (2 * p.pool_ls);
+    FE_CHECK(p.unit_stride && p.Cin % 32 == 0 && p.Kp == p.Cin && p.Cout % 64 == 0 && p.vec_epi && !p.res && p.batch <= 1 && p.act != ACT_PRELU &&
+                 p.pool_ls <= 3 && (!p.gate || p.gate_c1) && p.M % g == 0 && p.H == (p.pool_th << p.pool_ls) && p.W == (p.pool_tw << p.pool_ls) && !p.tapw,
+             "conv_dma: pooling epilogue preconditions");
+    launch_dma_variant<2, 2, 2, 1, 3, true>(p, s);
+    return;
+  }
+  if (p.tapw) {
+    FE_CHECK(p.Cout == 64 && p.vec_epi && !p.res && !p.gate && p.batch <= 1 && p.act != ACT_PRELU && p.ldy % 4 == 0 && p.ldy >= 4 && p.ldy <= 32 &&
+                 p.tap_t > 0 && p.tap_t <= p.ldy && p.tap_ld % 4 == 0 && p.tap_ld >= 64 && ((uintptr_t)p.tapw & 15) == 0,
+             "conv_dma: tap epilogue preconditions");
+    launch_dma_variant<2, 2, 2, 1, 4, false>(p, s);
+    return;
+  }
   if (p.act == ACT_PRELU) {
     FE_CHECK(p.slope, "conv_dma: PReLU without slopes");
     switch (tile) {
diff --git a/facet_amd/csrc/model_topiq.hip b/facet_amd/csrc/model_topiq.hip
--- a/facet_amd/csrc/model_topiq.hip
+++ b/facet_amd/csrc/model_topiq.hip
@@ -168,6 +168,39 @@
   linear_forward(c, w.lin1, t2, d, B * Lq, hbuf, ff, ACT_GELU);
   linear_forward(c, w.lin2, hbuf, ff, B * Lq, tgt, d, ACT_NONE, a, d);
   c.arena.rewind(mark);
+}
+
+Tensor topiq_gate_forward_f32(Ctx& c, const GatedConvW& g, const Tensor& f, int th, int tw, int wblk_act, int gate_act) {
+  const bool fuse_pool = getenv("FE_NO_FUSED_POOL_F32") == nullptr, fuse_tap = getenv("FE_NO_FUSED_TAP_F32") == nullptr;
+  const bool pool = f.h > th && f.w > tw;
+  Tensor out = pool ? c.arena.tensor(f.n, th, tw, g.split_x1.Cout) : c.arena.tensor(f.n, f.h, f.w, g.split_x1.Cout);
+  const size_t mark = c.arena.mark();
+  ConvOpts o0; o0.act = wblk_act;
+  Tensor wa = conv_new(c, g.w0, f, o0);
+  ConvOpts o2; o2.act = wblk_act; o2.ph = o2.pw = 1;
+  ConvOpts o4; o4.act = ACT_SIGMOID; o4.ph = o4.pw = 1;
+  Tensor wc;
+  if (fuse_tap && conv_tap_fusable(c, g.w2, o2, g.w4, o4, wa)) {
+    wc = c.arena.tensor(wa.n, wa.h, wa.w, g.w4.Cout);
+    conv_tap_forward(c, g.w2, o2, g.w4, o4, wa, wc);
+  } else {
+    Tensor wb = conv_new(c, g.w2, wa, o2);
+    wc = conv_new(c, g.w4, wb, o4);
+  }
+  ConvOpts og; og.act = gate_act; og.gate = &wc;
+  if (pool && fuse_pool) {
+    Tensor full;
+    full.n = f.n; full.h = f.h; full.w = f.w; full.c = full.ld = g.split_x1.Cout;
+    og.pool = &out;
+    conv_forward(c, g.split_x1, f, full, og);
+  } else if (pool) {
+    Tensor gated = conv_new(c, g.split_x1, f, og);
+    launch_adaptive_avgpool(gated, out, c.stream);
+  } else {
+    conv_forward(c, g.split_x1, f, out, og);
+  }
+  c.arena.rewind(mark);
+  return out;
 }
 
 template <class T>
@@ -210,40 +243,45 @@
         continue;
       }
     }
-    ConvOptsT<T> o0; o0.act = m.wblk_act;
-    TensorT<T> wa = conv_new(c, g.w0, f, o0);
-    ConvOptsT<T> o2; o2.act = m.wblk_act; o2.ph = o2.pw = 1;
-    TensorT<T> wb;
-    bool tiled = false;
-    if constexpr (sizeof(T) == 2) {
-      if (g.w2_frag && wa.c == 64 && wa.ld == 64 && !g.w2.scale && wa.pixels() >= 131072 && !getenv("FE_NO_FUSED_C64")) {
-        wb = c.arena.tensor_t<T>(wa.n, wa.h, wa.w, 64);
-        const double flops = 2.0 * (double)wa.pixels() * 576.0 * 64;
-        hipEvent_t e0 = nullptr, e1 = nullptr;
-        if (c.profile) { FE_HIP(hipEventCreate(&e0)); FE_HIP(hipEventCreate(&e1)); FE_HIP(hipEventRecord(e0, c.stream)); }
-        launch_conv3x3_c64(wa, wb, (const TensorT<T>*)nullptr, g.w2_frag, nullptr, nullptr, g.w2.shift, nullptr, nullptr, m.wblk_act, c.stream);
-        if (c.profile) {
-          FE_HIP(hipEventRecord(e1, c.stream)); FE_HIP(hipEventSynchronize(e1));
-          float ms = 0.f;
-          FE_HIP(hipEventElapsedTime(&ms, e0, e1));
-          (void)hipEventDestroy(e0); (void)hipEventDestroy(e1);
-          char nm[128];
-          snprintf(nm, sizeof nm, "%s halo-tiled conv3x3 64->64 M=%d", PrecOf<T>::value == PREC_F16 ? "f16" : "bf16", (int)wa.pixels());
-          c.timings.push_back({nm, flops, 2.0 * (double)wa.pixels() * 128, ms});
+    TensorT<T> gated;
+    if constexpr (sizeof(T) == 4) {
+      gated = topiq_gate_forward_f32(c, g, f, th, tw, m.wblk_act, m.gate_act);
+    } else {
+      ConvOptsT<T> o0; o0.act = m.wblk_act;
+      TensorT<T> wa = conv_new(c, g.w0, f, o0);
+      ConvOptsT<T> o2; o2.act = m.wblk_act; o2.ph = o2.pw = 1;
+      TensorT<T> wb;
+      bool tiled = false;
+      if constexpr (sizeof(T) == 2) {
+        if (g.w2_frag && wa.c == 64 && wa.ld == 64 && !g.w2.scale && wa.pixels() >= 131072 && !getenv("FE_NO_FUSED_C64")) {
+          wb = c.arena.tensor_t<T>(wa.n, wa.h, wa.w, 64);
+          const double flops = 2.0 * (double)wa.pixels() * 576.0 * 64;
+          hipEvent_t e0 = nullptr, e1 = nullptr;
+          if (c.profile) { FE_HIP(hipEventCreate(&e0)); FE_HIP(hipEventCreate(&e1)); FE_HIP(hipEventRecord(e0, c.stream)); }
+          launch_conv3x3_c64(wa, wb, (const TensorT<T>*)nullptr, g.w2_frag, nullptr, nullptr, g.w2.shift, nullptr, nullptr, m.wblk_act, c.stream);
+          if (c.profile) {
+            FE_HIP(hipEventRecord(e1, c.stream)); FE_HIP(hipEventSynchronize(e1));
+            float ms = 0.f;
+            FE_HIP(hipEventElapsedTime(&ms, e0, e1));
+            (void)hipEventDestroy(e0); (void)hipEventDestroy(e1);
+            char nm[128];
+            snprintf(nm, sizeof nm, "%s halo-tiled conv3x3 64->64 M=%d", PrecOf<T>::value == PREC_F16 ? "f16" : "bf16", (int)wa.pixels());
+            c.timings.push_back({nm, flops, 2.0 * (double)wa.pixels() * 128, ms});
+          }
+          c.flops_accum += flops; c.flops_half += flops;
+          tiled = true;
         }
-        c.flops_accum += flops; c.flops_half += flops;
-        tiled = true;
       }
-    }
-    if (!tiled) wb = conv_new(c, g.w2, wa, o2);
-    ConvOptsT<T> o4; o4.act = ACT_SIGMOID; o4.ph = o4.pw = 1;
-    TensorT<T> wc = conv_new(c, g.w4, wb, o4);
-    ConvOptsT<T> og; og.act = m.gate_act; og.gate = &wc;
-    TensorT<T> gated = conv_new(c, g.split_x1, f, og);
-    if (gated.h > th && gated.w > tw) {
-      TensorT<T> pooled = c.arena.tensor_t<T>(B, th, tw, gated.c);
-      launch_adaptive_avgpool(gated, pooled, c.stream);
-      gated = pooled;
+      if (!tiled) wb = conv_new(c, g.w2, wa, o2);
+      ConvOptsT<T> o4; o4.act = ACT_SIGMOID; o4.ph = o4.pw = 1;
+      TensorT<T> wc = conv_new(c, g.w4, wb, o4);
+      ConvOptsT<T> og; og.act = m.gate_act; og.gate = &wc;
+      gated = conv_new(c, g.split_x1, f, og);
+      if (gated.h > th && gated.w > tw) {
+        TensorT<T> pooled = c.arena.tensor_t<T>(B, th, tw, gated.c);
+        launch_adaptive_avgpool(gated, pooled, c.stream);
+        gated = pooled;
+      }
     }
     FE_CHECK(gated.h == th && gated.w == tw, "topiq head: level %d is %dx%d, expected %dx%d", i, gated.h, gated.w, th, tw);
     TensorT<T> t = mat_view(tok[i], B * L, d, d);
diff --git a/include/facet_engine.h b/include/facet_engine.h
--- a/include/facet_engine.h
+++ b/include/facet_engine.h
@@ -98,6 +98,9 @@
 int fe_op_topiq_gate64(fe_ctx* ctx, const float* x, int n, int h, int w, const float* w0, const float* b0, const float* w2,
                        const float* b2, const float* w4, float b4, const float* wx, const float* bx, int wblk_act,
                        int gate_act, float* y);
+int fe_op_topiq_gate_f32(fe_ctx* ctx, const float* x, int n, int c, int h, int w, const float* w0, const float* b0, const float* w2,
+                         const float* b2, const float* w4, float b4, const float* wx, const float* bx, int wblk_act,
+                         int gate_act, int ho, int wo, float* y);
 int fe_op_conv3x3_c64(fe_ctx* ctx, const float* x, int n, int h, int w, const float* w2, const float* scale2,
                       const float* shift2, int act2, const float* w3, const float* scale3, const float* shift3,
                       const float* res, float* y);
```

Measured after the change: 232.9 (median of 6 runs). 1.7% higher.
